# sanazkaviani/3d-latent-diffusion-model

Hardware: AMD Instinct MI355X
Metric: UNet denoising steps/sec (bf16, 1x4x24x24x24 latent; whole job = sum over GPUs) (higher is better)
Workload: dtype bf16

## Files before the change

### 3d-latent-diffusion-model_amd/_lib.py

```python
from __future__ import annotations

import ctypes as C
import os
import threading

LDM_MAX_LEVELS = 8
_HERE = os.path.dirname(os.path.abspath(__file__))
LIB_PATH = os.environ.get("LDM3D_LIB") or os.path.join(_HERE, "libldm3d.so")


class UNetCfg(C.Structure):
    _fields_ = [("spatial_dims", C.c_int), ("in_channels", C.c_int), ("out_channels", C.c_int),
                ("num_levels", C.c_int),
                ("channels", C.c_int * LDM_MAX_LEVELS), ("attention_levels", C.c_int * LDM_MAX_LEVELS),
                ("num_head_channels", C.c_int * LDM_MAX_LEVELS), ("num_res_blocks", C.c_int * LDM_MAX_LEVELS),
                ("norm_num_groups", C.c_int), ("norm_eps", C.c_float)]


class VaeCfg(C.Structure):
    _fields_ = [("spatial_dims", C.c_int), ("in_channels", C.c_int), ("out_channels", C.c_int),
                ("latent_channels", C.c_int), ("num_levels", C.c_int),
                ("channels", C.c_int * LDM_MAX_LEVELS), ("num_res_blocks", C.c_int * LDM_MAX_LEVELS),
                ("attention_levels", C.c_int * LDM_MAX_LEVELS),
                ("norm_num_groups", C.c_int), ("norm_eps", C.c_float),
# ... 139 lines not shown
    "ldm_op_conv3d_fin_gn": (C.c_int, [_P, C.c_int, _P, _P, _P, C.c_int, _P, _P, _P, C.c_int, C.c_float, C.c_int, _P, _P,
                                       C.c_int, C.c_int, C.c_int, C.c_int, C.c_int, C.c_int, C.c_int, C.c_int, _P, C.c_size_t, _P]),
    "ldm_op_group_norm_scratch_bytes": (C.c_size_t, [C.c_int, C.c_int, C.c_int]),
    "ldm_op_group_norm": (C.c_int, [_P, C.c_int, _P, C.c_int, _P, _P, C.c_int, C.c_float, C.c_int, _P, C.c_int, C.c_int,
                                    _P, C.c_size_t, _P]),
    "ldm_op_attention": (C.c_int, [_P, _P, C.c_int, C.c_int, C.c_int, _P]),
    "ldm_op_attention_hd": (C.c_int, [_P, _P, _P, C.c_int, C.c_int, C.c_int, C.c_int, _P]),
    "ldm_op_attention_bwd_hd": (C.c_int, [_P, _P, _P, _P, _P, _P, C.c_int, C.c_int, C.c_int, C.c_int, _P]),
    "ldm_op_attention_train": (C.c_int, [_P, _P, _P, C.c_int, C.c_int, C.c_int, _P]),
    "ldm_op_attention_bwd": (C.c_int, [_P, _P, _P, _P, _P, _P, C.c_int, C.c_int, C.c_int, _P]),
    "ldm_profile_start": (C.c_int, [C.c_int, C.c_int, C.c_int, C.c_int]),
    "ldm_profile_detail": (C.c_int, [C.POINTER(C.c_double), C.POINTER(C.c_double), C.c_int]),
    "ldm_profile_stop": (C.c_int, [C.POINTER(C.c_double)]),
    "ldm_set_plan_trace": (C.c_int, [C.c_char_p]),
    "ldm_op_pack_ncdhw_f32": (C.c_int, [_P, _P, C.c_int, C.c_int, C.c_int, C.c_int64, _P]),
    "ldm_op_unpack_ndhwc_f32": (C.c_int, [_P, _P, C.c_int, C.c_int, C.c_int, C.c_int64, _P]),
    "ldm_op_im2col_f32": (C.c_int, [_P, _P] + [C.c_int] * 10 + [_P]),
    "ldm_op_col2im_f32": (C.c_int, [_P, _P] + [C.c_int] * 10 + [_P]),
    "ldm_op_leaky_relu_f32": (C.c_int, [_P, _P, C.c_int64, C.c_float, _P]),
    "ldm_op_leaky_relu_bwd_f32": (C.c_int, [_P, _P, _P, C.c_int64, C.c_float, _P]),
    "ldm_op_gemm_f32": (C.c_int, [_P, C.c_int, _P, _P, _P, C.c_int64, C.c_int, C.c_int, C.c_int, _P]),
    "ldm_debug_conv_block_slots": (C.c_int, [C.c_int]),
    "ldm_op_conv3d_block_stats_rows": (C.c_int, [C.c_int, C.c_int, C.c_int, C.c_int]),
    "ldm_op_conv3d_block": (C.c_int, [_P, C.c_int, _P, _P, _P, C.c_int, _P, _P, _P, C.c_int, C.c_int, C.c_int, C.c_int, C.c_int, _P]),
    "ldm_op_conv3d_block128": (C.c_int, [_P, C.c_int, _P, _P, _P, C.c_int, _P, _P, _P, C.c_int, C.c_int, C.c_int, C.c_int, _P]),
    "ldm_op_linear_bf16": (C.c_int, [_P, C.c_int, _P, C.c_int, _P, _P, _P, _P, _P, C.c_int64, C.c_int, C.c_int, C.c_int, C.c_int,
                                     _P, C.c_int, C.c_int, _P, _P, C.c_int, C.c_float, C.c_int, _P, _P]),
    "ldm_op_linear_f32x3": (C.c_int, [_P, C.c_int, _P, C.c_int, _P, _P, _P, _P, _P, C.c_int64, C.c_int, C.c_int, C.c_int, _P]),
    "ldm_op_gemm_wgrad_f32": (C.c_int, [_P, C.c_int, _P, C.c_int, _P, C.c_int, C.c_int64, C.c_int, _P]),
    "ldm_op_group_norm_f32_scratch_bytes": (C.c_size_t, [C.c_int, C.c_int, C.c_int, C.c_int]),
    "ldm_op_group_norm_f32": (C.c_int, [_P, C.c_int, _P, _P, C.c_int, C.c_float, C.c_int, _P, C.c_int, C.c_int, _P, C.c_size_t, _P]),
    "ldm_op_group_norm_bwd_f32": (C.c_int, [_P, _P, C.c_int, _P, _P, C.c_int, C.c_float, C.c_int, _P, _P, _P, C.c_int, C.c_int, _P, C.c_size_t, _P]),
    "ldm_op_conv3d_f32_stats_blocks": (C.c_int, [C.c_int, C.c_int, C.c_int, C.POINTER(C.c_int)]),
    "ldm_op_conv3d_f32": (C.c_int, [_P, C.c_int, _P, C.c_int, _P, _P, _P, C.c_int, _P, _P, C.c_int, _P, _P] + [C.c_int] * 13
                          + [_P, C.c_size_t, _P]),
    "ldm_op_weight_flip_transpose_f32_ws_bytes": (C.c_size_t, [C.c_int, C.c_int, C.c_int]),
    "ldm_op_weight_flip_transpose_f32": (C.c_int, [_P, _P] + [C.c_int] * 6 + [_P, C.c_size_t, _P]),
    "ldm_op_conv3d_wgrad_f32": (C.c_int, [_P, C.c_int, _P, C.c_int, _P] + [C.c_int] * 13 + [_P]),
    "ldm_op_attention_f32": (C.c_int, [_P, _P, _P] + [C.c_int] * 5 + [_P]),
    "ldm_op_attention_bwd_f32": (C.c_int, [_P] * 6 + [C.c_int] * 4 + [_P]),
    "ldm_op_group_norm_bwd2_f32": (C.c_int, [_P, _P, C.c_int, _P, C.c_int, _P, _P, C.c_int, C.c_float, C.c_int, _P, _P, _P, _P, _P, _P,
                                             C.c_int, C.c_int, _P, C.c_size_t, _P]),
    "ldm_op_upsample_bwd_f32": (C.c_int, [_P, _P] + [C.c_int] * 5 + [_P]),
    "ldm_op_group_norm_bwd_saved_scratch_bytes": (C.c_size_t, [C.c_int] * 4),
    "ldm_op_group_norm_bwd_fold_chunks": (C.c_int, [C.c_int] * 4),
    "ldm_op_group_norm_bwd_saved": (C.c_int, [_P, _P, C.c_int, _P, C.c_int, _P, _P, _P, C.c_int, C.c_int] + [_P] * 7
                                    + [C.c_int] * 3 + [_P, C.c_size_t, _P]),
    "ldm_op_colsum_finalize_ws_bytes": (C.c_size_t, [_P, C.c_int]),
    "ldm_op_colsum_finalize": (C.c_int, [_P, _P, _P, C.c_int, C.c_int, _P, C.c_size_t, _P]),
    "ldm_op_grad_export_ws_bytes": (C.c_size_t, [_P, C.c_int]),
    "ldm_op_grad_export": (C.c_int, [_P, _P, _P, C.c_int, C.c_int, _P, C.c_size_t, _P]),
    "ldm_op_weight_flip_transpose_batched_ws_bytes": (C.c_size_t, [_P, C.c_int]),
    "ldm_op_weight_flip_transpose_batched": (C.c_int, [_P, _P, _P, C.c_int, _P, C.c_size_t, _P]),
    "ldm_op_linear_bwd_nz": (C.c_int, [C.c_int]),
    "ldm_op_linear_bwd": (C.c_int, [_P] * 6 + [C.c_int] * 6 + [_P, C.c_size_t, _P]),
    "ldm_op_upsample_bwd": (C.c_int, [_P, _P] + [C.c_int] * 5 + [_P]),
    "ldm_op_add_bf16": (C.c_int, [_P, _P, _P, C.c_int64, _P]),
    "ldm_op_vae_heads": (C.c_int, [_P] * 5 + [C.c_int] * 3 + [_P]),
    "ldm_op_vae_heads_bwd": (C.c_int, [_P, C.c_int] + [_P] * 5 + [C.c_int] * 5 + [_P]),
    "ldm_debug_kstamps": (C.c_int, [C.POINTER(C.c_uint64), C.c_int, C.c_int]),
    "ldm_model_plan_conv_cfgs": (C.c_int, [_P, C.c_char_p, C.c_int, C.c_int, C.c_int, C.c_int, C.POINTER(C.c_int), C.c_int]),
    "ldm_comm_unique_id": (C.c_int, [C.c_char_p]),
    "ldm_comm_init": (C.c_int, [C.c_int, C.c_int, C.c_char_p, C.POINTER(_P)]),
    "ldm_comm_init_custom": (C.c_int, [C.c_int, C.c_int, _P, _P, C.POINTER(_P)]),
    "ldm_comm_allreduce": (C.c_int, [_P, _P, C.c_int64, C.c_int, C.c_int, _P]),
    "ldm_comm_broadcast": (C.c_int, [_P, _P, C.c_int64, C.c_int, C.c_int, _P]),
    "ldm_comm_barrier": (C.c_int, [_P, _P]),
    "ldm_comm_destroy": (None, [_P]),
    "ldm_comm_rank": (C.c_int, [_P]),
    "ldm_comm_world": (C.c_int, [_P]),
    "ldm_model_set_grad_sync": (C.c_int, [_P, _P]),
    "ldm_model_set_grad_wire": (C.c_int, [_P, C.c_int]),
    "ldm_model_grad_sync_pending": (C.c_int, [_P]),
    "ldm_comm_stats": (C.c_int, [_P, C.POINTER(C.c_int64)]),
    "ldm_comm_is_rccl": (C.c_int, [_P]),
    "ldm_comm_rccl_version": (C.c_int, []),
    "ldm_model_plan_launches": (C.c_int, [_P, C.c_char_p, C.c_int, C.c_int, C.c_int, C.c_int]),
    "ldm_model_grad_sync_trace": (C.c_int, [_P, C.POINTER(C.c_double), C.POINTER(C.c_double), C.POINTER(C.c_int64), C.c_int]),
    "ldm_model_grad_schedule": (C.c_int, [_P, C.c_int, C.c_int, C.c_int, C.c_int, C.POINTER(C.c_int), C.POINTER(C.c_int64),
                                          C.POINTER(C.c_int64), C.POINTER(C.c_int), C.c_int]),
    "ldm_op_conv3d_thin": (C.c_int, [_P, C.c_int, _P, _P, _P] + [C.c_int] * 6 + [_P]),
    "ldm_op_conv3d_thin_f32_ws_bytes": (C.c_size_t, [C.c_int] * 6),
    "ldm_op_conv3d_thin_f32": (C.c_int, [_P, C.c_int, _P, _P, _P] + [C.c_int] * 6 + [_P, C.c_size_t, _P]),
    "ldm_op_timestep_embedding": (C.c_int, [_P, _P, C.c_int, C.c_int, _P]),
    "ldm_op_gemv": (C.c_int, [_P, C.c_int, _P, _P, _P] + [C.c_int] * 6 + [_P]),
    "ldm_op_pack2": (C.c_int, [_P, C.c_int, _P, C.c_int, _P, C.c_int, C.c_int, C.c_int64, C.c_int, C.c_int, C.c_float, _P]),
    "ldm_op_pack_im2col": (C.c_int, [_P, C.c_int, _P, C.c_int, _P] + [C.c_int] * 6 + [C.c_float, _P]),
    "ldm_op_phase_weights": (C.c_int, [_P, _P, C.c_int, C.c_int, _P]),
    "ldm_op_im2col_weights": (C.c_int, [_P, _P, C.c_int, C.c_int, C.c_int, C.c_int, _P]),
    "ldm_op_x3_weights": (C.c_int, [_P, _P, C.c_int64, C.c_int, _P]),
    "ldm_op_x3_phase_weights": (C.c_int, [_P, _P, C.c_int, C.c_int, _P]),
    "ldm_op_split_f32": (C.c_int, [_P, _P] + [C.c_int] * 6 + [_P]),
}
ALLREDUCE_FN = C.CFUNCTYPE(C.c_int, _P, _P, C.c_int64, C.c_int, C.c_int, _P)

_lib = None
_lock = threading.Lock()


class LdmError(RuntimeError):
    """Raised for every non-zero ldm_status (message from ldm_last_error)."""


def lib() -> C.CDLL:
    global _lib
    if _lib is None:
        with _lock:
            if _lib is None:
                if not os.path.exists(LIB_PATH):
                    raise LdmError(f"{LIB_PATH} not found: build it with `python -c 'import __graft_entry__ as g; "
                                   f"g.build()'` or `make -C {os.path.join(_HERE, 'csrc')}` (no CPU fallback exists)")
                h = C.CDLL(LIB_PATH)
                for name, (res, args) in SIGNATURES.items():
                    fn = getattr(h, name)
                    fn.restype = res
                    fn.argtypes = args
                _lib = h
    return _lib


def check(status: int) -> None:
    if status != 0:
        msg = lib().ldm_last_error()
        raise LdmError(f"libldm3d status {status}: {msg.decode() if msg else '?'}")


def ptr(t) -> int | None:
    return None if t is None else t.data_ptr()


def current_stream() -> int:
    import torch
    return torch.cuda.current_stream().cuda_stream
```

### 3d-latent-diffusion-model_amd/csrc/ldm3d.hip

```cpp
#include <hip/hip_runtime.h>
#include <dlfcn.h>
#include <math.h>
#include <stdarg.h>
#include <stdio.h>
#include <stdlib.h>
#include <string.h>

#include <algorithm>
#include <atomic>
#include <map>
#include <memory>
#include <string>
#include <type_traits>
#include <vector>

#include "../../include/ldm3d.h"
#include "attention.h"
#include "conv_igemm.h"
#include "conv_halo.h"
#include "conv_cube.h"
#include "conv_plane.h"
#ifdef LDM_EXPERIMENTS
#include "conv_halo_pp.h"
#include "conv_halo_rw.h"
// ... 51 lines not shown
        BLK_ATTR(8, 0, true)
#endif
#ifdef LDM_BLOCK_EXPERIMENTS
        BLK_ATTR(8, 1, false) BLK_ATTR(8, 2, false) BLK_ATTR(8, 4, false) BLK_ATTR(8, 3, false) BLK_ATTR(8, 7, false) BLK_ATTR(8, 8, false) BLK_ATTR(8, 15, false)
#endif
#undef BLK_ATTR
        attr_set = true;
    }
    const unsigned grid = (unsigned)tiles;
#ifdef LDM_BLOCK_EXPERIMENTS
#define BLK_DBG(D) if (TH == 8 && dbg == D) { hipLaunchKernelGGL((conv3_block_kernel<8, D, false>), dim3(grid), dim3(256), BlkGeom<8>::LDS_ALL, s, q); return hipGetLastError(); }
    BLK_DBG(1) BLK_DBG(2) BLK_DBG(4) BLK_DBG(3) BLK_DBG(7) BLK_DBG(8) BLK_DBG(15)
#undef BLK_DBG
#endif
    (void)dbg; (void)persist;
#ifdef LDM_EXPERIMENTS
    const long slots = g_block_slots > 0 ? g_block_slots : 2L * cus_tab[dev_];
    if (TH == 8 && persist && tiles > slots) { hipLaunchKernelGGL((conv3_block_kernel<8, 0, true>), dim3((unsigned)slots), dim3(256), BlkGeom<8>::LDS_ALL, s, q); return hipGetLastError(); }
#endif
    if (TH == 8) hipLaunchKernelGGL((conv3_block_kernel<8, 0, false>), dim3(grid), dim3(256), BlkGeom<8>::LDS_ALL, s, q);
    else hipLaunchKernelGGL((conv3_block_kernel<4, 0, false>), dim3(grid), dim3(256), BlkGeom<4>::LDS_ALL, s, q);
    return hipGetLastError();
}
static int device_cus() {
    static int tab[32] = {};
    int d = 0; if (hipGetDevice(&d) != hipSuccess || d < 0 || d >= 32) return 256;
    if (!tab[d]) { hipDeviceProp_t pr; tab[d] = (hipGetDeviceProperties(&pr, d) == hipSuccess && pr.multiProcessorCount >= 8) ? pr.multiProcessorCount : 256; }
    return tab[d];
}
static hipError_t launch_conv_block128(const BlockParams& q0, hipStream_t s) {
    BlockParams q = q0;
    q.td = (q.D + BLK_TD - 1) / BLK_TD; q.th = (q.H + 7) / 8; q.tw = (q.W + BLK_TW - 1) / BLK_TW;
    static bool attr_tab[32] = {}; bool& attr_set = attr_flag(attr_tab);
    if (!attr_set) {
        hipError_t e = hipFuncSetAttribute(reinterpret_cast<const void*>(&conv3_block128_kernel), hipFuncAttributeMaxDynamicSharedMemorySize, Blk128::LDS_ALL);
        if (e != hipSuccess) return e;
        attr_set = true;
    }
    hipLaunchKernelGGL(conv3_block128_kernel, dim3((unsigned)((long)q.N * q.td * q.th * q.tw)), dim3(512), Blk128::LDS_ALL, s, q);
    return hipGetLastError();
}
static inline int rup(int v, int m) { return (v + m - 1) / m * m; }
static inline size_t rup_sz(size_t v, size_t m) { return (v + m - 1) / m * m; }

static inline uint16_t host_f2bf(float f) {
    uint32_t u; memcpy(&u, &f, 4);
    if ((u & 0x7fffffffu) > 0x7f800000u) return (uint16_t)((u >> 16) | 0x40);
    u += 0x7fffu + ((u >> 16) & 1u);
    return (uint16_t)(u >> 16);
}

enum BaseId { BASE_NULL = 0, BASE_WS, BASE_W, BASE_IO0, BASE_IO1, BASE_IO2, BASE_IO3, BASE_IO4, BASE_IO5, BASE_W32, BASE_TAPO, BASE_TAPI, BASE_TTAB, BASE_SST, BASE_COUNT };
struct Ref { int base = BASE_NULL; size_t off = 0; };
static inline Ref ws_ref(size_t off) { Ref r; r.base = BASE_WS; r.off = off; return r; }
static inline Ref w_ref(size_t off) { Ref r; r.base = BASE_W; r.off = off; return r; }
static inline Ref io_ref(int i) { Ref r; r.base = BASE_IO0 + i; r.off = 0; return r; }
static inline Ref w32_ref(size_t off) { Ref r; r.base = BASE_W32; r.off = 2 * off; return r; }

struct Act {
    size_t off = 0; int C = 0; int N = 0, D = 0, H = 0, W = 0; bool valid = false;
    size_t stats_off = 0; bool has_stats = false;
    int stats_nrb = 0;
    int esz = 2;
    bool hl = false;
    size_t cs_off = 0; int cs_rows = 0;
    size_t bytes() const { return (size_t)N * D * H * W * C * esz; }
    long rows() const { return (long)N * D * H * W; }
};

enum OpKind { OP_PACK, OP_CONV, OP_FINALIZE, OP_GN_STATS, OP_GN_FINALIZE, OP_GN_PREP, OP_GN_APPLY, OP_ATTN, OP_SINUSOID,
              OP_GEMV, OP_VAE_HEADS, OP_GN_FUSED,
              OP_WT , OP_WT_BATCH, OP_WGRAD, OP_EXPORT , OP_EXPORT_BATCH, OP_COLSUM, OP_GNB, OP_ATTN_BWD, OP_ADD, OP_SUMPOOL, OP_LIN_DX, OP_LIN_DW, OP_VAE_HEADS_BWD,
              OP_GEMM_LIGHT,
              OP_COLSUM_BATCH,
              OP_IM2COL,
              OP_PACK32, OP_CONV32, OP_FIN32, OP_GN_STATS32, OP_GN_APPLY32, OP_ATTN32, OP_GEMV32,
              OP_TAP,
              OP_BUCKET, OP_BUCKET_JOIN,
              OP_UPS_SPLIT32,
              OP_CONV_THIN,
              OP_FIN_GN,
              OP_GEMM_LIGHT32,
              OP_CONV_BLOCK,
              OP_TEMB_ROW };

struct ConvCfg { int wgm, wgn, bk, splitk; int halo = 0, mtps = 0, qps = 0; int slab_lg = 0; int cube = 0; int th = 0, big = 0; int plane = 0; int wg = 0; };

struct ConvRec {
    Ref xa, xb, w; int ca, cb;
    Ref x1a, x1b, w1; int c1a, c1b;
    int N, Din, Hin, Win, Dout, Hout, Wout;
    int k, stride, pad, M;
    int couts, cout_pad, cout_real;
    int nchunk0, nchunk1, mtiles, ntiles;
    bool ups, exact;
    bool phase;
    bool x3;
    bool ep32_ndhwc, ep32_ncdhw;
    Ref bias, bias2, temb, residual; int temb_stride;
    Ref out; int f32_out;
    Ref partial, stats;
    int stats_nrb, stats_rows;
    Ref gamma, beta, gn_out; int gn_groups, gn_silu, gn_lg; float gn_eps;
    Ref gn_stats; int gn_nrb;
};

struct GnRec {
    Ref xa, xb; int ca, cb, N, DHW;
    Ref gamma, beta; int groups; float eps; bool silu;
    Ref stats_a, stats_b; int nrb_a, nrb_b;
    Ref partial; int nslab, rows_per_slab;
    Ref ab, mr;
    Ref out; bool out_hl;
    int rows_per_block, chunks;
    Ref dy, gsum, dgamma_n, dbeta_n;
    Ref cs; bool leaves_colsums;
    Ref acc_a, acc_b, dxa, dxb;
    int dgamma_flat, dbeta_flat;
    bool fp32;
    int count, out_stride; bool over_n;
};

struct WgradRec {
    Ref dy, x, dw; int cdy, cx;
    int Cout, Cin, dw_ld, dw_ci_off;
    int N, Din, Hin, Win, Dout, Hout, Wout;
    int ksize, stride, pad, ups, M;
    int ksplit, rows_total;
    bool fp32;
};

struct LayoutRec {
    Ref a, b, dst;
    int N, c_real, c_stored, D, H, W, DHW;
    bool internal;
    int esz, mode, ups;
    bool guided;
};

struct AttnRec {
    Ref qkv, out, lse;
    Ref d_o, delta, dqkv;
    int B, N, C, heads, d; float scale;
    bool x3, fp32;
};

struct LinRec {
    Ref w, bias, x, y;
    Ref dy, x_pre, dx, dW, db, part;
    int B, I, O, x_stride, y_stride, dy_stride;
    int silu, nz; bool fp32;
};

struct ElemRec {
    Ref a, b, out; int n;
    Ref ml, noise, mu, sigma, z;
    Ref dz, g_mu, g_sigma, dy; int c_dz;
    int N, D, H, W, C, L, DHW;
    bool fp32;
};

struct RangeRec { int first, end, count; bool fp32; };

struct Op {
    OpKind kind;
    ConvCfg cc;
    ConvRec cv;
    GnRec gn;
    WgradRec wg;
    LayoutRec lay;
    AttnRec at;
    LinRec lin;
    ElemRec el;
    RangeRec rg;
};

struct Pool {
    struct Blk { size_t off, size; };
    std::vector<Blk> free_list;
    std::map<size_t, size_t> live;
    size_t top = 0, high = 0;
    size_t alloc(size_t bytes) {
        bytes = rup_sz(bytes, 256);
// ... 191 lines not shown
        ConvW o = new_conv_slot(C, C, 1);
        reg_conv_into(p + ".attn.out_proj", o, C, C, 1, 0, true);
        convs[p + ".attn.out_proj"] = o;
    }
};

static int wgrad_ksplit(long M, int taps, int cout, int cin, bool hp = false, int stride = 1, int ups = 0);
static void conv32_cfg(long M, int cout_pad, int steps, bool x3, int* bn_out, int* sk_out);
static int fin32_stats_blocks(int N, int dhwo, int couts, int* rows);

static void gn_slabs(int N, int C, int DHW, int vec, int max_slabs, int* nslab, int* rps) {
    const int rows_par = std::max(1, 256 / std::max(1, C / vec));
    const int ns = std::min((DHW + rows_par - 1) / rows_par, std::max(1, max_slabs / N));
    *rps = (DHW + ns - 1) / ns;
    *nslab = (DHW + *rps - 1) / *rps;
}
static int gn_row_chunks(int N, int C, int DHW, int blocks, int row_multiple, int* rpb) {
    const int slices = (C + 63) / 64;
    const int chunks = std::max(1, std::min(blocks / (slices * N), (DHW + row_multiple - 1) / row_multiple));
    *rpb = rup((DHW + chunks - 1) / chunks, row_multiple);
    return (DHW + *rpb - 1) / *rpb;
}
static int gn_fused_blocks() { static const int v = ldm_xknob("LDM_GN_BLOCKS", 512); return v; }
static int gnb_fold_chunks(int N, int C, int groups, int DHW, int nslab, int* rpb) {
    if (C / groups > 64 || nslab > 512) return 0;
    return gn_row_chunks(N, C, DHW, 256, 32, rpb);
}
static int lin_dx_nz(int O) { return std::max(1, std::min(64, O / 64)); }
static int conv_out_size(int in, int k, int stride, int pad, int ups) {
    return ((in << ups) + ((stride == 2 && pad == 0 && k == 3) ? 1 : 2 * pad) - k) / stride + 1;
}
static int conv_mtiles(const ConvRec& c, const ConvCfg& cc) {
    const int bm = 64 * cc.wgm;
    if (cc.halo) return c.N * cc.mtps;
    if (c.phase) return c.N * 8 * (int)(((long)c.Din * c.Hin * c.Win + bm - 1) / bm);
    return (c.M + bm - 1) / bm;
}
static int splitk_stats_rows(int N, int dhw) { return N == 1 ? (dhw + 31) / 32 : dhw % 32 ? 0 : dhw / 32; }
static int conv_stats_rows(const ConvRec& c, const ConvCfg& cc) {
    const int dhwo = c.Dout * c.Hout * c.Wout, bm = 64 * cc.wgm;
    if (cc.splitk > 1) return splitk_stats_rows(c.N, dhwo);
    if (cc.plane) return c.Dout;
    if (cc.halo || c.phase) return conv_mtiles(c, cc) / c.N;
    return c.N == 1 ? (c.M + bm - 1) / bm : dhwo % bm ? 0 : dhwo / bm;
}

struct Builder {
    ldm_model* m; Plan* plan; Pool pool;
    size_t partial_off = 0, partial_bytes = 0;
    size_t gnpart_off = 0, gnpart_bytes = 0;
    size_t gnab_off = 0, gnab_bytes = 0;
    std::vector<size_t> partial_fixups, gnpart_fixups, gnab_fixups;
    std::string err;

    Act new_act(int N, int D, int H, int W, int C) {
        Act a; a.N = N; a.D = D; a.H = H; a.W = W; a.C = C; a.valid = true; a.esz = hp ? 4 : 2; a.off = pool.alloc(a.bytes()); return a;
    }
    bool hp = false;
    int tap_mode = 0;
    void tap(const std::string& name, Act& h, int c_real) {
        if (!tap_mode) return;
        TapInfo t; t.name = name; t.dims[0] = h.N; t.dims[1] = c_real; t.dims[2] = h.D; t.dims[3] = h.H; t.dims[4] = h.W; t.off = plan->tap_elems;
        plan->tap_elems += (size_t)h.N * c_real * h.D * h.H * h.W;
        Op o{}; o.kind = OP_TAP; LayoutRec& l = o.lay; l.a = ws_ref(h.off);
        l.dst.base = BASE_TAPO; l.dst.off = t.off * 4; l.b.base = BASE_TAPI; l.b.off = t.off * 4;
        l.N = h.N; l.c_real = c_real; l.c_stored = h.C; l.DHW = h.D * h.H * h.W; l.esz = h.esz; l.mode = tap_mode;
        plan->ops.push_back(o);
        plan->taps.push_back(t);
        if (tap_mode == 2 && h.has_stats) { pool.release(h.stats_off); h.has_stats = false; }
    }
    void pack(Ref src_a, Ref src_b, const Act& dst, int c_real, bool internal) {
        Op o{}; o.kind = hp ? OP_PACK32 : OP_PACK; LayoutRec& l = o.lay; l.a = src_a; l.b = src_b; l.dst = ws_ref(dst.off);
        l.N = dst.N; l.c_real = c_real; l.c_stored = dst.C; l.DHW = dst.D * dst.H * dst.W; l.internal = internal;
        l.guided = guided && !internal;
        plan->ops.push_back(o);
    }
    void free_act(Act& a) {
        if (train) return;
        if (a.valid) { pool.release(a.off); if (a.has_stats) pool.release(a.stats_off); }
        a.valid = false; a.has_stats = false;
    }
    bool train = false, recording = false;
    bool guided = false;

    struct ConvArgs {
        Act xa, xb;
        const ConvW* w = nullptr;
        int k = 3, stride = 1, pad = 1, ups = 0;
        int Do = 0, Ho = 0, Wo = 0;
        Act g1a, g1b; const ConvW* w1 = nullptr;
        Ref temb; int temb_stride = 0;
        Act residual;
        bool f32_out = false; Ref out_ref; int cout_real = 0;
        bool want_stats = true;
        Ref w_over; bool no_bias = false; int exact = 0;
        int temb_row = -1;
        int f32_tag = 0;
        const GnW* pre_gn = nullptr; int pre_groups = 0, pre_nrb = 0; float pre_eps = 0.f;
    };
    struct Tape {
        int kind = 0;
        ConvArgs c; Act out; bool leaf_input = false;
        const GnW* g = nullptr; Act xa, xb; size_t ab_off = 0, mr_off = 0; int groups = 0; bool silu = false;
        Act qkv, o; size_t lse_off = 0; int head_ch = 64;
    };
    std::vector<Tape> tape;

    static bool halo_enabled() { return ldm_knob("LDM_CONV_HALO", 1) != 0; }
    static int tall_mode() { return ldm_xknob("LDM_HALO_TALL", 2); }
    static bool light_enabled() { return ldm_knob("LDM_GEMM_LIGHT", 1) != 0; }
    static bool two_wg_enabled() { return ldm_knob("LDM_IGEMM_2WG", 1) != 0; }
    static bool phase_enabled() { return ldm_knob("LDM_CONV_PHASE", 1) != 0; }
    static bool halo_skip_enabled() { static const int v = ldm_knob("LDM_HALO_SKIP", 1); return v != 0; }
    static bool halo_skip_split_enabled() { static const int v = ldm_knob("LDM_HALO_SKIP_SPLIT", 1); return v != 0; }
    static bool cube_enabled() { return ldm_knob("LDM_CONV_CUBE", 1) != 0; }
    static bool cube_ok(int D, int H, int W, int cin0, int c1a, int c1b, int cout_pad) {
        return cube_enabled() && D >= 1 && H >= 1 && W >= 1 && D <= CUBE_EDGE && H <= CUBE_EDGE && W <= CUBE_EDGE && cin0 % 64 == 0 && cin0 >= 128 &&
               c1a % 64 == 0 && c1b % 64 == 0 && cout_pad % 16 == 0;
    }
    static ConvCfg cube_cfg(int cin0) { ConvCfg c{2, 2, 64, cin0 / 64}; c.cube = 1; return c; }
    static bool plane_enabled() { return ldm_knob("LDM_CONV_PLANE", 1) != 0; }
    static int plane_max_cin() { return (int)ldm_knob("LDM_CONV_PLANE_MAX_CIN", 256); }
    static bool plane_ok(int D, int H, int W, int cin0, int c1a, int c1b, int cout_pad) {
        return plane_enabled() && D >= 1 && H >= 1 && W >= 1 && D <= PLANE_EDGE && H <= PLANE_EDGE && W <= PLANE_EDGE &&
               (D > CUBE_EDGE || H > CUBE_EDGE || W > CUBE_EDGE) && cin0 % 64 == 0 && cin0 >= 128 && cin0 <= plane_max_cin() &&
               c1a % 64 == 0 && c1b % 64 == 0 && cout_pad % 16 == 0;
    }
    static ConvCfg plane_cfg() { ConvCfg c{2, 2, 64, 1}; c.plane = 1; return c; }
    static ConvCfg choose_cfg(long M, int cout_pad, int steps0, int bk, int halo_n = 0, long halo_dhw = 0, bool halo_only = false, int steps1 = 0) {
        ConvCfg best{2, 2, bk, 1}; double best_t = 1e30;
        const int steps = steps0 + steps1;
        const int rb = bk * 2;
        static const int splits[] = {1, 2, 3, 4, 6, 8, 9, 12, 16, 18, 24, 27, 32, 48, 64};
        for (int wgn = 1; wgn <= 4 && !halo_only; wgn *= 2) {
            const int bn = 64 * wgn, bm = 64 * (4 / wgn);
            if (cout_pad % bn) continue;
            const long tiles = ((M + bm - 1) / bm) * (cout_pad / bn);
            const double c_mfma = (double)bm * bn * bk * 2.0 / 4096.0;
            const double c_load = (double)(bm + bn) * rb / 28.0;
            const double c_step = std::max(c_mfma, c_load) + 60.0;
            for (int sk : splits) {
                if (sk > 1 && steps / sk < 6) break;
                const long nwg = tiles * sk;
                const int sps = (steps + sk - 1) / sk;
                const double rounds = ceil((double)nwg / 256.0);
                double t = rounds * (sps * c_step + 2500.0);
                if (sk > 1) t += 6000.0 + (double)M * cout_pad * 4.0 * sk * 2.0 / 2500.0;
                if (t < best_t) { best_t = t; best = ConvCfg{4 / wgn, wgn, bk, sk}; }
            }
        }
        if (halo_n > 0 && bk == 64 && cout_pad % 128 == 0 && halo_enabled()) {
            const int mtps = (int)((halo_dhw + 125) / 126), Q = steps0 / 3;
            const long tiles = (long)halo_n * mtps * (cout_pad / 128);
            const double c_mfma = 128.0 * 128.0 * 64.0 * 2.0 / 4096.0;
            const double c_load = (128.0 / 3.0 + 128.0) * 128.0 / 28.0;
            const double c_step = std::max(c_mfma, c_load) + 30.0;
            for (int sk : splits) {
                if (sk > 1 && Q / sk < 3) break;
                const int qps = (Q + sk - 1) / sk, skr = (Q + qps - 1) / qps;
                const long nwg = tiles * skr;
                const double rounds = ceil((double)nwg / 256.0);
                double t = rounds * (3.0 * qps * c_step + 2500.0 + ((steps1 + skr - 1) / skr) * 1.6 * c_step + (steps1 && skr > 1 ? 800.0 : 0.0));
                if (skr > 1) t += 6000.0 + (double)M * cout_pad * 4.0 * skr * 2.0 / 2500.0;
                if (steps1 && skr > 1 && !halo_skip_split_enabled()) continue;
                if (t < best_t) { best_t = t; best = ConvCfg{2, 2, 64, skr}; best.halo = 1; best.mtps = mtps; best.qps = qps; }
            }
        }
        if (halo_n > 0 && bk == 64 && cout_pad % 64 == 0 && halo_enabled() && tall_mode() != 0) {
            const int mtps = (int)((halo_dhw + 253) / 254), Q = steps0 / 3;
            const long tiles = (long)halo_n * mtps * (cout_pad / 64);
            const double c_mfma = 256.0 * 64.0 * 64.0 * 2.0 / 4096.0;
            const double c_load = (256.0 / 3.0 + 64.0) * 128.0 / 28.0;
            const double c_step = std::max(c_mfma, c_load) + 30.0;
            for (int sk : splits) {
                if (sk > 1 && Q / sk < 3) break;
                const int qps = (Q + sk - 1) / sk, skr = (Q + qps - 1) / qps;
                const long nwg = tiles * skr;
                const double rounds = ceil((double)nwg / 256.0);
                double t = rounds * (3.0 * qps * c_step + 2500.0 + ((steps1 + skr - 1) / skr) * 1.6 * c_step + (steps1 && skr > 1 ? 800.0 : 0.0));
                if (skr > 1) t += 6000.0 + (double)M * cout_pad * 4.0 * skr * 2.0 / 2500.0;
                if (steps1 && skr > 1 && !halo_skip_split_enabled()) continue;
                if (tall_mode() == 2 && cout_pad % 128 == 0) t = 1e31;
                if (tall_mode() == 3 && skr == 1 && best.halo == 1 && best.splitk == 1) t = 0.0;
                if (t < best_t) { best_t = t; best = ConvCfg{4, 1, 64, skr}; best.halo = 2; best.mtps = mtps; best.qps = qps; }
            }
        }
        return best;
    }
    static bool conv_halo_ok(const ConvRec& c, int bk, int forced_split) {
        return c.k == 3 && c.stride == 1 && c.pad == 1 && !c.ups && !c.exact && c.cb == 0 && bk == 64 &&
               c.Din == c.Dout && c.Hin == c.Hout && c.Win == c.Wout &&
               (c.c1a + c.c1b == 0 || (halo_skip_enabled() && (forced_split <= 1 || halo_skip_split_enabled())));
    }
    static void two_wg_steps(ConvCfg& cc, int steps, long mtiles, int cout_pad) {
        if (!cc.halo && !cc.plane && cc.bk == 64 && cc.wgm <= 2 && cc.splitk == 1 && two_wg_enabled() && steps <= 64 &&
            mtiles * (cout_pad / (64 * cc.wgn)) >= 512) cc.bk = 32;
    }
    static ConvCfg pick_cfg(const ConvRec& c, int bk, bool cube, bool plane, int wgn = 0, int splitk = 0) {
        const int cin0 = c.ca + c.cb, steps0 = c.k * c.k * c.k * (cin0 / bk), steps1 = (c.c1a + c.c1b) / bk;
        const long dhwo = (long)c.Dout * c.Hout * c.Wout;
        const bool halo_ok = conv_halo_ok(c, bk, splitk);
        ConvCfg cc = choose_cfg(c.M, c.cout_pad, steps0, bk, halo_ok ? c.N : 0, dhwo, false, steps1);
        if (cube && halo_ok && cube_ok(c.Dout, c.Hout, c.Wout, cin0, c.c1a, c.c1b, c.cout_pad)) cc = cube_cfg(cin0);
        else if (plane && halo_ok && plane_ok(c.Dout, c.Hout, c.Wout, cin0, c.c1a, c.c1b, c.cout_pad)) cc = plane_cfg();
        if (wgn) {
            const bool halo = halo_ok && halo_enabled();
            cc.wgn = wgn; cc.wgm = 4 / wgn; cc.halo = (wgn == 2 && halo && c.cout_pad % 128 == 0) ? 1 : (wgn == 1 && halo && tall_mode() != 0) ? 2 : 0;
        }
        if (splitk) cc.splitk = splitk;
        if (cc.halo) {
            const int Q = steps0 / 3;
            cc.qps = (Q + std::min(cc.splitk, Q) - 1) / std::min(cc.splitk, Q); cc.splitk = (Q + cc.qps - 1) / cc.qps;
            cc.mtps = (int)((dhwo + (cc.halo == 2 ? 253 : 125)) / (cc.halo == 2 ? 254 : 126));
        }
        if (!wgn && !splitk) two_wg_steps(cc, steps0 + steps1, conv_mtiles(c, cc), c.cout_pad);
        return cc;
    }

    static ConvRec conv_rec(const ConvArgs& a, int k, int stride, int pad, long M, int cout_real) {
        ConvRec c{}; c.N = a.xa.N; c.Din = a.xa.D; c.Hin = a.xa.H; c.Win = a.xa.W; c.Dout = a.Do; c.Hout = a.Ho; c.Wout = a.Wo;
        c.k = k; c.stride = stride; c.pad = pad; c.M = (int)M; c.couts = rup(a.w->cout, 32); c.cout_pad = a.w->cout_pad; c.cout_real = cout_real;
        return c;
    }
    static void conv_epilogue(ConvRec& c, const ConvArgs& a, const Act& out) {
        c.bias = a.no_bias ? Ref() : w_ref(a.w->b_off); c.temb = a.temb; c.temb_stride = a.temb_stride;
        c.residual = a.residual.valid ? ws_ref(a.residual.off) : Ref();
        c.out = a.f32_out ? a.out_ref : ws_ref(out.off); c.f32_out = a.f32_out ? 1 : 0;
    }
    static void conv_sources(ConvRec& c, const ConvArgs& a) {
        c.xa = ws_ref(a.xa.off); c.xb = a.xb.valid ? ws_ref(a.xb.off) : Ref(); c.ca = a.xa.C; c.cb = a.xb.valid ? a.xb.C : 0;
    }
    void record_conv(const ConvArgs& a, const Act& out) { if (recording) { Tape t; t.kind = 0; t.c = a; t.out = out; tape.push_back(t); } }
    static long thin_tiles(const ConvArgs& a) {
        return (long)a.xa.N * ((a.Do + THIN_TD - 1) / THIN_TD) * ((a.Ho + THIN_TH - 1) / THIN_TH) * ((a.Wo + THIN_TW - 1) / THIN_TW);
    }
    void emit_thin(const ConvArgs& a, long M, Ref w, int cout_real, bool x3) {
        Op op{}; op.kind = OP_CONV_THIN;
        ConvRec& c = op.cv; c = conv_rec(a, 3, 1, 1, M, cout_real); conv_epilogue(c, a, Act());
        c.xa = ws_ref(a.xa.off); c.ca = x3 ? 2 * a.xa.C : a.xa.C; c.x3 = x3; c.w = w;
        plan->ops.push_back(op);
    }
    Act emit_light(OpKind kind, const ConvArgs& a, long M, Ref w, int big, bool want_stats) {
        const int N = a.xa.N, rows = big ? 64 : 32;
        Op op{}; op.kind = kind; op.cc.big = big;
        ConvRec& c = op.cv; c = conv_rec(a, a.k, a.stride, a.pad, M, a.w->cout);
        op.cc.wg = kind == OP_GEMM_LIGHT && gemm_wg_ok(!a.xb.valid, a.xa.C + (a.xb.valid ? a.xb.C : 0), M);
        if (a.pre_gn) {
            op.cc.wg = 2; c.gamma = w_ref(a.pre_gn->g_off); c.beta = w_ref(a.pre_gn->b_off); c.gn_groups = a.pre_groups; c.gn_eps = a.pre_eps;
            c.gn_stats = ws_ref(a.xa.stats_off); c.gn_nrb = a.pre_nrb;
        }
        Act out = new_act(N, a.Do, a.Ho, a.Wo, c.couts);
        const long dhwo = (long)a.Do * a.Ho * a.Wo;
        if (want_stats && (N == 1 || dhwo % rows == 0)) {
            out.stats_off = pool.alloc((size_t)((M + rows - 1) / rows) * c.couts * 2 * 4); out.has_stats = true;
            out.stats_nrb = (int)(N == 1 ? (M + rows - 1) / rows : dhwo / rows);
        }
        conv_epilogue(c, a, out); conv_sources(c, a); c.w = w; c.stats = out.has_stats ? ws_ref(out.stats_off) : Ref();
        plan->ops.push_back(op);
        record_conv(a, out);
        return out;
    }
    Act emit_conv_block(const ConvArgs& a, long M, int th, int tiles) {
        const int N = a.xa.N;
        Op op{}; op.kind = OP_CONV_BLOCK; op.cc.th = th;
        ConvRec& c = op.cv; c = conv_rec(a, 3, 1, 1, M, a.w->cout);
        Act out = new_act(N, a.Do, a.Ho, a.Wo, c.couts);
        if (a.want_stats) { out.stats_off = pool.alloc((size_t)N * tiles * c.couts * 2 * 4); out.has_stats = true; out.stats_nrb = tiles; }
        conv_epilogue(c, a, out); conv_sources(c, a);
        c.w = a.w_over.base != BASE_NULL ? a.w_over : w_ref(a.w->w_off); c.stats = out.has_stats ? ws_ref(out.stats_off) : Ref();
        plan->ops.push_back(op);
        record_conv(a, out);
        return out;
    }
    void fin32_stats(Op& f, Act& out, const ConvArgs& a, int N, int dhwo, int couts) {
        static const int on = ldm_xknob("LDM_FIN32_STATS", 1);
        if (!on || train || !a.want_stats || a.f32_out || couts % 4 || couts > 1024) return;
        int rows = 0;
        const int nrb = fin32_stats_blocks(N, dhwo, couts, &rows);
        out.stats_off = pool.alloc((size_t)N * nrb * couts * 2 * 4); out.has_stats = true; out.stats_nrb = nrb;
        f.cv.stats = ws_ref(out.stats_off); f.cv.stats_nrb = nrb; f.cv.stats_rows = rows;
    }
    void fin32_x3(const ConvArgs& a, Act& out, int C, long M, int splitk, int ntiles) {
        Op f{}; f.kind = OP_FIN32; f.cc = ConvCfg{2, 2, 32, splitk};
        ConvRec& d = f.cv; d = conv_rec(a, 3, 1, 1, M, a.f32_out && a.cout_real ? a.cout_real : a.w->cout);
        conv_epilogue(d, a, out);
        d.w = w32_ref(a.w->w_off); d.ca = C; d.nchunk0 = C / 32; d.ntiles = ntiles; d.mtiles = (int)((M + 127) / 128);
        fin32_stats(f, out, a, a.xa.N, a.Do * a.Ho * a.Wo, d.couts);
        partial_fixups.push_back(plan->ops.size()); plan->ops.push_back(f);
    }
    Act conv32(const ConvArgs& a, const std::string& tag) {
        const ConvW& w = *a.w;
        if (a.w1) { err = "fp32 precision: unsupported conv form (" + tag + ")"; return Act(); }
        const int cin0 = a.xa.C + (a.xb.valid ? a.xb.C : 0);
        if (cin0 != w.cin_s || cin0 % 16 || a.xa.C % 16) { err = "conv " + tag + ": channel bookkeeping mismatch"; return Act(); }
        const int N = a.xa.N;
        const long M = (long)N * a.Do * a.Ho * a.Wo;
        if (M >= (1L << 31)) { err = "conv " + tag + ": M too large"; return Act(); }
        {
            static const int x3_phase = ldm_xknob("LDM_X3_PHASE", 1);
            const int C = a.xa.C;
            if (x3_phase && !train && a.ups == 1 && !a.exact && a.k == 3 && a.stride == 1 && a.pad == 1 && !a.xb.valid && !a.w1 && !a.f32_out &&
                a.w_over.base == BASE_NULL && !a.xa.hl && a.Do == 2 * a.xa.D && a.Ho == 2 * a.xa.H && a.Wo == 2 * a.xa.W && phase_enabled() &&
                w.x3p_off != (size_t)-1 && x3_halo_ok(w, M, C) && a.temb.base == BASE_NULL && !a.residual.valid) {
                Act sp = new_act(N, a.xa.D, a.xa.H, a.xa.W, C); sp.hl = true;
                Op u{}; u.kind = OP_UPS_SPLIT32; u.lay.a = ws_ref(a.xa.off); u.lay.dst = ws_ref(sp.off);
                u.lay.N = N; u.lay.c_stored = C; u.lay.D = a.xa.D; u.lay.H = a.xa.H; u.lay.W = a.xa.W; u.lay.ups = 0;
                plan->ops.push_back(u);
                Op op{}; op.kind = OP_CONV;
                ConvRec& c = op.cv; c = conv_rec(a, 2, 1, 1, M, w.cout);
                c.xa = ws_ref(sp.off); c.xb = ws_ref(sp.off); c.w = Ref{BASE_W32, 2 * m->arena_bytes + w.x3p_off};
                c.ca = 2 * C; c.cb = C; c.phase = c.x3 = true;
                const int steps0 = 8 * (3 * C / 64);
                ConvCfg cc = choose_cfg(M, w.cout_pad, steps0, 64);
                if (cc.wgm > 2 || cc.splitk != 1) cc = ConvCfg{2, 2, 64, 1};
                if (w.cout_pad % (64 * cc.wgn)) cc = ConvCfg{4, 1, 64, 1};
                two_wg_steps(cc, steps0, conv_mtiles(c, cc), w.cout_pad);
                op.cc = cc; c.nchunk0 = 3 * C / cc.bk;
                Act out = new_act(N, a.Do, a.Ho, a.Wo, rup(w.cout, 32));
                partial_bytes = std::max(partial_bytes, (size_t)M * w.cout_pad * 4);
                partial_fixups.push_back(plan->ops.size()); plan->ops.push_back(op);
                fin32_x3(a, out, C, M, 1, 1);
                free_act(sp);
// ... 43 lines not shown
                return out;
            }
            if (cc.splitk == 1 && x3_fused) {
                c.ep32_ndhwc = true; conv_epilogue(c, a, out);
                if (a.want_stats) {
                    out.stats_nrb = conv_stats_rows(c, cc);
                    out.stats_off = pool.alloc((size_t)N * out.stats_nrb * couts * 2 * 4); out.has_stats = true; c.stats = ws_ref(out.stats_off);
                }
                plan->ops.push_back(op);
                return out;
            }
            partial_bytes = std::max(partial_bytes, (size_t)cc.splitk * M * w.cout_pad * 4);
            partial_fixups.push_back(plan->ops.size()); plan->ops.push_back(op);
            fin32_x3(a, out, C, M, cc.splitk, w.cout_pad / 128 ? w.cout_pad / 128 : 1);
            return out;
        }
        static const int f32_x3 = ldm_knob("LDM_F32_X3", 1);
        const bool x3 = (f32_x3 == 2 || (f32_x3 == 1 && !train)) && cin0 % 32 == 0 && a.xa.C % 32 == 0;
        {
            static const int light_x3 = ldm_xknob("LDM_LIGHT_X3", 1);
            static const long light_x3_max_m = ldm_xknob("LDM_LIGHT_X3_MAX_M", 4096L);
            if (light_x3 && x3 && M <= light_x3_max_m && a.k == 1 && a.stride == 1 && a.pad == 0 && !a.ups && !a.exact && !a.f32_out && !a.xa.hl && a.temb.base == BASE_NULL &&
                (!a.xb.valid || a.xb.C % 32 == 0) && w.cout_pad % 32 == 0 && a.xa.D == a.Do && a.xa.H == a.Ho && a.xa.W == a.Wo &&
                M * (long)std::max(cin0, w.cout_pad) * 4 < (1L << 31)) {
                return emit_light(OP_GEMM_LIGHT32, a, M, a.w_over.base != BASE_NULL ? a.w_over : w32_ref(w.w_off), gemm_light_x3_big(M, w.cout_pad),
                                  a.want_stats && !train);
            }
        }
        const int kb = x3 ? 32 : 16;
        const int taps = a.k * a.k * a.k, nchunk = cin0 / kb, steps = taps * nchunk;
        const int mtiles = (int)((M + 127) / 128);
        int bn = 0, sk = 0;
        conv32_cfg(M, w.cout_pad, steps, x3, &bn, &sk);
        const int ntiles = (w.cout_pad + bn - 1) / bn;
        const int couts = a.f32_out ? 0 : rup(w.cout, 32);
        Act out;
        if (!a.f32_out) out = new_act(N, a.Do, a.Ho, a.Wo, couts);
        Op op{}; op.kind = OP_CONV32; op.cc = ConvCfg{2, bn / 64, kb, sk};
        ConvRec& c = op.cv; c = conv_rec(a, a.k, a.stride, a.pad, M, a.cout_real ? a.cout_real : w.cout);
        conv_epilogue(c, a, out); conv_sources(c, a);
        c.w = a.w_over.base != BASE_NULL ? a.w_over : w32_ref(w.w_off);
        c.ups = a.ups & 1; c.exact = a.exact & 1; c.nchunk0 = nchunk; c.mtiles = mtiles; c.ntiles = ntiles;
        if (sk > 1) { partial_bytes = std::max(partial_bytes, (size_t)sk * M * w.cout_pad * 4); partial_fixups.push_back(plan->ops.size()); }
        plan->ops.push_back(op);
        if (sk > 1) { Op f = op; f.kind = OP_FIN32; fin32_stats(f, out, a, N, a.Do * a.Ho * a.Wo, couts); partial_fixups.push_back(plan->ops.size()); plan->ops.push_back(f); }
        record_conv(a, out);
        return out;
    }

    Act conv(const ConvArgs& a, std::string tag = "") {
        if (hp) return conv32(a, tag);
        const ConvW& w = *a.w;
        const int cin0 = a.xa.C + (a.xb.valid ? a.xb.C : 0);
        int bk = 64;
        if (a.xa.C % 64 || (a.xb.valid && a.xb.C % 64)) bk = 32;
        int cin1 = 0;
        if (a.w1) {
            cin1 = a.g1a.C + (a.g1b.valid ? a.g1b.C : 0);
            if (a.g1a.C % 64 || (a.g1b.valid && a.g1b.C % 64)) bk = 32;
        }
        if (cin0 != w.cin_s || (a.w1 && cin1 != a.w1->cin_s) || cin0 % 32 || cin1 % 32) {
            err = "conv " + tag + ": channel bookkeeping mismatch"; return Act();
        }
        const int N = a.xa.N;
        const long M = (long)N * a.Do * a.Ho * a.Wo;
        {
            const long rows0 = (long)N * a.xa.D * a.xa.H * a.xa.W;
            const long big = std::max(std::max(rows0 * a.xa.C, a.xb.valid ? rows0 * a.xb.C : 0L),
                                      a.w1 ? std::max(M * a.g1a.C, a.g1b.valid ? M * a.g1b.C : 0L) : 0L) * 2;
            if (big >= (1L << 32)) { err = "conv " + tag + ": a source tensor exceeds 4 GiB (split the batch)"; return Act(); }
        }
        {
            static const int thin = ldm_knob("LDM_CONV_THIN", 1);
            static const long thin_min = ldm_knob("LDM_CONV_THIN_MIN", 512L);
            const int cr = a.cout_real ? a.cout_real : w.cout;
            if (thin && a.f32_out && a.k == 3 && a.stride == 1 && a.pad == 1 && !a.ups && !a.exact && !a.xb.valid && !a.w1 &&
                a.temb.base == BASE_NULL && !a.residual.valid && a.w_over.base == BASE_NULL && cr <= 4 && cin0 % 32 == 0 && cin0 <= 128 &&
                a.xa.D == a.Do && a.xa.H == a.Ho && a.xa.W == a.Wo &&
                thin_tiles(a) >= thin_min) {
                emit_thin(a, M, w_ref(w.w_off), cr, false);
                record_conv(a, Act());
                return Act();
            }
        }
        const bool phase = a.ups == 1 && !a.exact && a.k == 3 && a.stride == 1 && a.pad == 1 && !train && !a.xb.valid && !a.w1 &&
                           a.w_over.base == BASE_NULL && w.wp_off != 0 && phase_enabled() &&
                           a.Do == 2 * a.xa.D && a.Ho == 2 * a.xa.H && a.Wo == 2 * a.xa.W;
        if (gemm_light_ok(a.k, a.stride, a.ups, cin0, !a.w1, !a.f32_out && a.temb.base == BASE_NULL) && light_enabled() &&
            a.xa.D == a.Do && a.xa.H == a.Ho && a.xa.W == a.Wo && M * (long)cin0 * 2 < (1L << 31))
            return emit_light(OP_GEMM_LIGHT, a, M, a.w_over.base != BASE_NULL ? a.w_over : w_ref(w.w_off), gemm_light_big(M, w.cout_pad), a.want_stats);
        if (a.pre_gn) { err = "conv " + tag + ": a GroupNorm prologue needs the light GEMM"; return Act(); }
        if (conv_block_enabled() && a.k == 3 && a.stride == 1 && a.pad == 1 && a.ups == 0 && !a.exact && !a.xb.valid && !a.w1 && !a.f32_out &&
            w.cout_pad == 64 && rup(w.cout, 32) == 64 && cin0 <= conv_block_max_cin() &&
            a.xa.D == a.Do && a.xa.H == a.Ho && a.xa.W == a.Wo) {
            const int TH = conv_block_th();
            const int td = (a.Do + BLK_TD - 1) / BLK_TD, th = (a.Ho + TH - 1) / TH, tw = (a.Wo + BLK_TW - 1) / BLK_TW;
            static const long min_blocks = ldm_knob("LDM_CONV_BLOCK_MIN", 512L);
            if ((long)N * td * th * tw >= min_blocks) return emit_conv_block(a, M, TH, td * th * tw);
        }
        if (conv_block128_enabled() && a.k == 3 && a.stride == 1 && a.pad == 1 && a.ups == 0 && !a.exact && !a.xb.valid && !a.w1 && !a.f32_out &&
            w.cout_pad == 128 && rup(w.cout, 32) == 128 && cin0 <= conv_block128_max_cin() && a.xa.D == a.Do && a.xa.H == a.Ho && a.xa.W == a.Wo) {
            const int td = (a.Do + BLK_TD - 1) / BLK_TD, th = (a.Ho + 7) / 8, tw = (a.Wo + BLK_TW - 1) / BLK_TW;
            static const long min_blocks = ldm_knob("LDM_CONV_BLOCK128_MIN", 192L);
            static const long max_blocks = ldm_xknob("LDM_CONV_BLOCK128_MAX", 0L);
            const long tiles128 = (long)N * td * th * tw;
            if (tiles128 >= min_blocks && tiles128 <= (max_blocks > 0 ? max_blocks : (long)device_cus())) return emit_conv_block(a, M, 8, td * th * tw);
        }
        if (M >= (1L << 31)) { err = "conv " + tag + ": M too large"; return Act(); }
        Op op{}; op.kind = OP_CONV;
        ConvRec& c = op.cv; c = conv_rec(a, phase ? 2 : a.k, a.stride, a.pad, M, a.cout_real ? a.cout_real : w.cout);
        conv_sources(c, a);
        c.w = a.w_over.base != BASE_NULL ? a.w_over : w_ref(phase ? w.wp_off : w.w_off);
        if (a.w1) {
            c.x1a = ws_ref(a.g1a.off); c.c1a = a.g1a.C; c.w1 = w_ref(a.w1->w_off); c.bias2 = w_ref(a.w1->b_off);
            if (a.g1b.valid) { c.x1b = ws_ref(a.g1b.off); c.c1b = a.g1b.C; }
        }
        c.phase = phase; c.ups = !phase && (a.ups & 1); c.exact = !phase && (a.exact & 1);
        const ConvCfg cc = op.cc = pick_cfg(c, bk, !train && !phase, !train && !phase && !a.f32_out);
        c.nchunk0 = cin0 / cc.bk; c.nchunk1 = cin1 / cc.bk;
        Act out;
        if (!a.f32_out) {
            out = new_act(N, a.Do, a.Ho, a.Wo, c.couts);
            const int nrb = a.want_stats ? conv_stats_rows(c, cc) : 0;
            if (a.want_stats && cc.splitk > 1) { out.stats_off = pool.alloc((size_t)((M + 31) / 32) * c.couts * 2 * 4); out.has_stats = true; }
            else if (nrb > 0) { out.stats_off = pool.alloc((size_t)N * nrb * c.couts * 2 * 4); out.has_stats = true; out.stats_nrb = nrb; }
        }
        conv_epilogue(c, a, out);
        c.stats = out.has_stats ? ws_ref(out.stats_off) : Ref();
        if (cc.splitk > 1) { partial_bytes = std::max(partial_bytes, (size_t)cc.splitk * M * w.cout_pad * 4); partial_fixups.push_back(plan->ops.size()); }
        plan->ops.push_back(op);
        if (cc.splitk > 1) { Op f = op; f.kind = OP_FINALIZE; partial_fixups.push_back(plan->ops.size()); plan->ops.push_back(f); }
        record_conv(a, out);
        return out;
    }

    static bool fin_gn_enabled() { static const int v = ldm_knob("LDM_FIN_GN", 1); return v != 0; }
    std::map<size_t, Act> prenorm;
    bool fuse_fin_gn(Act& raw, bool keep_raw, const GnW& g, int groups, float eps, bool silu, Act* y) {
        if (hp || train || !fin_gn_enabled() || plan->ops.size() < 2 || !raw.valid) return false;
        Op& f = plan->ops.back();
        Op& cv = plan->ops[plan->ops.size() - 2];
        if (f.kind != OP_FINALIZE || cv.kind != OP_CONV || f.cv.f32_out || f.cv.out.base != BASE_WS || f.cv.out.off != raw.off) return false;
        const int C = raw.C, N = raw.N, DHW = raw.D * raw.H * raw.W;
        if (C != g.C || !fin_gn_ok(C, groups, DHW) || f.cv.phase) return false;
        const int lg = fin_gn_lg(C, groups);
        static const long max_kb = ldm_knob("LDM_FIN_GN_MAX_KB", 400);
        if ((long)cv.cc.splitk * DHW * (C / groups) * 4 > max_kb * 1024) return false;
        if (f.cv.cout_pad % (1 << lg)) return false;
        Act out = new_act(N, raw.D, raw.H, raw.W, C);
        f.kind = OP_FIN_GN;
        f.cv.gamma = w_ref(g.g_off); f.cv.beta = w_ref(g.b_off); f.cv.gn_out = ws_ref(out.off);
        f.cv.stats = Ref();
        f.cv.gn_groups = groups; f.cv.gn_silu = silu ? 1 : 0; f.cv.gn_lg = lg; f.cv.gn_eps = eps;
        f.cc.slab_lg = lg; cv.cc.slab_lg = lg; cv.cv.stats = Ref();
        if (raw.has_stats) { pool.release(raw.stats_off); raw.has_stats = false; }
        if (!keep_raw) { f.cv.out = Ref(); pool.release(raw.off); raw.valid = false; }
        *y = out;
        return true;
    }

    static bool x3_halo_ok(const ConvW& w, long rows, int C) {
        static const int on = ldm_xknob("LDM_X3_HALO", 1);
        static const long min_rows = ldm_xknob("LDM_X3_HALO_ROWS", 1L);
        static const int f32_x3 = ldm_knob("LDM_F32_X3", 1);
        return on && f32_x3 != 0 && halo_enabled() && w.k == 3 && w.x3_off != (size_t)-1 && C == w.cin_s && C % 64 == 0 && rows >= min_rows &&
               rows * C * 4 < (1L << 32);
// ... 447 lines not shown

    size_t temb_all_off = 0; int tproj_stride = 0;

    void finish() {
        size_t top = rup_sz(pool.high, 256);
        partial_off = top; top += rup_sz(partial_bytes, 256);
        gnpart_off = top; top += rup_sz(gnpart_bytes, 256);
        gnab_off = top; top += rup_sz(gnab_bytes, 256);
        pool.high = top;
        for (size_t k : partial_fixups) plan->ops[k].cv.partial = ws_ref(partial_off);
        for (size_t k : gnpart_fixups) plan->ops[k].gn.partial = ws_ref(gnpart_off);
        for (size_t k : gnab_fixups) plan->ops[k].gn.ab = ws_ref(gnab_off);
        plan->ws_bytes = pool.high + 256;
    }
};

static int unet_register(ldm_model* m) {
    const ldm_unet_cfg& c = m->ucfg;
    const int L = c.num_levels; const int* ch = c.channels;
    const int temb = ch[0] * 4;
    for (int i = 0; i < L; ++i) if (ch[i] % 32 || ch[i] % c.norm_num_groups)
        return fail(LDM_ERR_UNSUPPORTED, "UNet channels must be multiples of 32 and of norm_num_groups (level %d: %d)", i, ch[i]);
    std::vector<std::pair<std::string, int>> tprojs;
    bool collect = true;
    auto reg_res = [&](const std::string& p, int cin, int cout) {
        if (collect) { tprojs.push_back({p, cout}); return; }
        m->reg_gn(p + ".norm1", cin);
        m->reg_conv(p + ".conv1", cin, cin, cout, 3);
        m->reg_gn(p + ".norm2", cout);
        m->reg_conv(p + ".conv2", cout, cout, cout, 3);
        if (cin != cout) m->reg_conv(p + ".skip_connection", cin, cin, cout, 1);
    };
    auto walk = [&]() {
    if (!collect) { m->reg_conv("conv_in", c.in_channels, rup(c.in_channels, 32), ch[0], 3); m->reg_im2col("conv_in", c.in_channels); }
    int oc = ch[0];
    for (int i = 0; i < L; ++i) {
        int ic = oc; oc = ch[i];
        for (int j = 0; j < c.num_res_blocks[i]; ++j) {
            char p[96]; snprintf(p, sizeof p, "down_blocks.%d.resnets.%d", i, j);
            reg_res(p, j == 0 ? ic : oc, oc);
            if (c.attention_levels[i] && !collect) { snprintf(p, sizeof p, "down_blocks.%d.attentions.%d", i, j); m->reg_attn(p, oc); }
        }
        if (i != L - 1 && !collect) { char p[96]; snprintf(p, sizeof p, "down_blocks.%d.downsampler.op", i); m->reg_conv(p, oc, oc, oc, 3); }
    }
    reg_res("middle_block.resnet_1", ch[L - 1], ch[L - 1]);
    if (!collect) m->reg_attn("middle_block.attention", ch[L - 1]);
    reg_res("middle_block.resnet_2", ch[L - 1], ch[L - 1]);
    oc = ch[L - 1];
    for (int i = 0; i < L; ++i) {
        const int lvl = L - 1 - i;
        int prev = oc; oc = ch[lvl];
        const int ic = ch[std::max(lvl - 1, 0)];
        const int nres = c.num_res_blocks[lvl] + 1;
        for (int j = 0; j < nres; ++j) {
            const int skip_c = (j == nres - 1) ? ic : oc;
            const int rin = (j == 0) ? prev : oc;
            char p[96]; snprintf(p, sizeof p, "up_blocks.%d.resnets.%d", i, j);
            reg_res(p, rin + skip_c, oc);
            if (c.attention_levels[lvl] && !collect) { snprintf(p, sizeof p, "up_blocks.%d.attentions.%d", i, j); m->reg_attn(p, oc); }
        }
        if (i != L - 1 && !collect) { char p[96]; snprintf(p, sizeof p, "up_blocks.%d.upsampler.postconv", i); m->reg_conv(p, oc, oc, oc, 3, true); }
    }
    if (!collect) { m->reg_gn("out.0", ch[0]); m->reg_conv("out.2", ch[0], ch[0], c.out_channels, 3); }
    };
    walk();
    m->reg_linear("time_embed.0", ch[0], temb);
    m->reg_linear("time_embed.2", temb, temb);
    int rows = 0; for (auto& t : tprojs) rows += t.second;
    m->tproj_rows = rows;
    m->tproj_w_off = m->arena_alloc((size_t)rows * temb * 2);
    m->tproj_b_off = m->arena_alloc((size_t)rows * 4);
    int r = 0;
    for (auto& t : tprojs) {
        m->tproj_row[t.first] = r;
        m->reg_linear_at(t.first + ".time_emb_proj", temb, t.second, m->tproj_w_off + (size_t)r * temb * 2, m->tproj_b_off + (size_t)r * 4);
        r += t.second;
    }
    collect = false;
    walk();
    return 0;
}

static int unet_build(ldm_model* m, int B, int D, int H, int W, Plan* plan, bool train, bool hp = false, int tap_mode = 0, bool temb_table = false,
                      bool guided = false) {
    const ldm_unet_cfg& c = m->ucfg;
    const int L = c.num_levels; const int* ch = c.channels;
    const int temb = ch[0] * 4, G = c.norm_num_groups; const float eps = c.norm_eps;
    if (train && tap_mode) return fail(LDM_ERR_UNSUPPORTED, "debug taps are inference-only");
    Builder b; b.m = m; b.plan = plan; b.train = train; b.recording = train; b.hp = hp; b.tap_mode = tap_mode; b.guided = guided;
    const size_t sin_off = b.pool.alloc((size_t)B * ch[0] * 4);
    const size_t e1_off = b.pool.alloc((size_t)B * temb * 4);
    const size_t e2_off = b.pool.alloc((size_t)B * temb * 4);
    b.tproj_stride = m->tproj_rows;
    b.temb_all_off = b.pool.alloc(((size_t)B * m->tproj_rows + 256) * 4);
    const LinW& l0 = m->lins.at("time_embed.0"); const LinW& l2 = m->lins.at("time_embed.2");
    if (temb_table && !train) {
        Op o{}; o.kind = OP_TEMB_ROW; o.lin.y = ws_ref(b.temb_all_off); o.lin.O = m->tproj_rows; o.lin.B = B; plan->ops.push_back(o);
    } else {
    { Op o{}; o.kind = OP_SINUSOID; o.lin.x = io_ref(2); o.lin.y = ws_ref(sin_off); o.lin.B = B; o.lin.O = ch[0];
      plan->ops.push_back(o); }
    auto gemv = [&](size_t w_off, size_t b_off, size_t x_off, size_t y_off, int I, int O, int xs, int ys, int silu) {
        Op o{}; o.kind = hp ? OP_GEMV32 : OP_GEMV; LinRec& l = o.lin;
        l.w = hp ? w32_ref(w_off) : w_ref(w_off); l.bias = w_ref(b_off); l.x = ws_ref(x_off); l.y = ws_ref(y_off);
        l.I = I; l.O = O; l.x_stride = xs; l.y_stride = ys; l.silu = silu; l.B = B; plan->ops.push_back(o);
    };
    gemv(l0.w_off, l0.b_off, sin_off, e1_off, ch[0], temb, ch[0], temb, 0);
    gemv(l2.w_off, l2.b_off, e1_off, e2_off, temb, temb, temb, temb, 1);
    gemv(m->tproj_w_off, m->tproj_b_off, e2_off, b.temb_all_off, temb, m->tproj_rows, temb, m->tproj_rows, 1);
    }

    const int cin_s = rup(c.in_channels, 32);
    Act h = b.conv_in_im2col("conv_in", io_ref(0), io_ref(1), B, D, H, W, c.in_channels, false);
    if (!h.valid) {
        if (!b.err.empty()) return fail(LDM_ERR_UNSUPPORTED, "%s", b.err.c_str());
        Act xin = b.new_act(B, D, H, W, cin_s);
        b.pack(io_ref(0), io_ref(1), xin, c.in_channels, false);
        h = b.conv3("conv_in", xin);
        if (train && !b.tape.empty()) b.tape.back().leaf_input = true;
        b.free_act(xin);
    }
    if (!h.valid) return fail(LDM_ERR_UNSUPPORTED, "%s", b.err.c_str());
    b.tap("conv_in", h, ch[0]);
    std::vector<Act> skips; skips.push_back(h);
    char p[96];
    for (int i = 0; i < L; ++i) {
        for (int j = 0; j < c.num_res_blocks[i]; ++j) {
            snprintf(p, sizeof p, "down_blocks.%d.resnets.%d", i, j);
            char pa[96]; snprintf(pa, sizeof pa, "down_blocks.%d.attentions.%d.norm", i, j);
            Act hn = b.resblock(p, h, Act(), ch[i], G, eps, ".skip_connection", true, c.attention_levels[i] ? &m->gns.at(pa) : nullptr);
            if (!hn.valid) return fail(LDM_ERR_UNSUPPORTED, "%s", b.err.c_str());
            b.tap(p, hn, ch[i]);
            if (c.attention_levels[i]) {
                snprintf(p, sizeof p, "down_blocks.%d.attentions.%d", i, j);
                Act ha = b.attention(p, hn, c.num_head_channels[i], G, eps);
                b.free_act(hn);
                if (!ha.valid) return fail(LDM_ERR_UNSUPPORTED, "%s", b.err.c_str());
                hn = ha;
                b.tap(p, hn, ch[i]);
            }
            skips.push_back(hn); h = hn;
        }
        if (i != L - 1) {
            if ((h.D | h.H | h.W) & 1) return fail(LDM_ERR_UNSUPPORTED, "odd spatial size %dx%dx%d at a UNet downsample", h.D, h.H, h.W);
            snprintf(p, sizeof p, "down_blocks.%d.downsampler.op", i);
            Act hd = b.conv3(p, h, 2, 1);
            if (!hd.valid) return fail(LDM_ERR_UNSUPPORTED, "%s", b.err.c_str());
            b.tap(p, hd, ch[i]);
            skips.push_back(hd); h = hd;
        }
    }
    {
        Act h1 = b.resblock("middle_block.resnet_1", h, Act(), ch[L - 1], G, eps, ".skip_connection", true, &m->gns.at("middle_block.attention.norm"));
        if (!h1.valid) return fail(LDM_ERR_UNSUPPORTED, "%s", b.err.c_str());
        b.tap("middle_block.resnet_1", h1, ch[L - 1]);
        Act h2 = b.attention("middle_block.attention", h1, c.num_head_channels[L - 1], G, eps);
        b.free_act(h1);
        if (!h2.valid) return fail(LDM_ERR_UNSUPPORTED, "%s", b.err.c_str());
        b.tap("middle_block.attention", h2, ch[L - 1]);
        Act h3 = b.resblock("middle_block.resnet_2", h2, Act(), ch[L - 1], G, eps, ".skip_connection", true);
        b.free_act(h2);
        if (!h3.valid) return fail(LDM_ERR_UNSUPPORTED, "%s", b.err.c_str());
        b.tap("middle_block.resnet_2", h3, ch[L - 1]);
        h = h3;
    }
    for (int i = 0; i < L; ++i) {
        const int lvl = L - 1 - i;
        for (int j = 0; j < c.num_res_blocks[lvl] + 1; ++j) {
            Act s = skips.back(); skips.pop_back();
            snprintf(p, sizeof p, "up_blocks.%d.resnets.%d", i, j);
            char pa[96]; snprintf(pa, sizeof pa, "up_blocks.%d.attentions.%d.norm", i, j);
            Act hn = b.resblock(p, h, s, ch[lvl], G, eps, ".skip_connection", true, c.attention_levels[lvl] ? &m->gns.at(pa) : nullptr);
            b.free_act(h); b.free_act(s);
// ... 189 lines not shown
    Act first = b.conv_in_im2col("encoder.blocks.0", io_ref(0), Ref(), B, D, H, W, c.in_channels, true);
    if (first.valid) {
        b.tap("encoder.blocks.0", first, c.channels[0]);
        LDM_TRY(vae_run_layout(b, "encoder", ae_encoder_layout(c), first, c.norm_num_groups, c.norm_eps, false, 0, &h, 1));
    } else {
        if (!b.err.empty()) return fail(LDM_ERR_UNSUPPORTED, "%s", b.err.c_str());
        Act xin = b.new_act(B, D, H, W, cs);
        b.pack(io_ref(0), Ref(), xin, c.in_channels, false);
        LDM_TRY(vae_run_layout(b, "encoder", ae_encoder_layout(c), xin, c.norm_num_groups, c.norm_eps, false, 0, &h));
    }
    const int dhw = h.D * h.H * h.W;
    const size_t ml_off = b.pool.alloc((size_t)B * 2 * c.latent_channels * dhw * 4);
    Builder::ConvArgs a; a.xa = h; a.w = &m->convs.at("quant_heads"); a.k = 1; a.pad = 0; a.Do = h.D; a.Ho = h.H; a.Wo = h.W;
    a.f32_out = true; a.out_ref = ws_ref(ml_off); a.cout_real = 2 * c.latent_channels;
    b.conv(a, "quant_heads");
    if (!b.err.empty()) return fail(LDM_ERR_UNSUPPORTED, "%s", b.err.c_str());
    b.free_act(h);
    { Op o{}; o.kind = OP_VAE_HEADS; ElemRec& e = o.el; e.ml = ws_ref(ml_off); e.noise = io_ref(1); e.mu = io_ref(2); e.sigma = io_ref(3); e.z = io_ref(4);
      e.N = B; e.L = c.latent_channels; e.DHW = dhw; plan->ops.push_back(o); }
    b.finish();
    return 0;
}

static int vae_build_decode(ldm_model* m, int B, int d, int h_, int w, Plan* plan, bool hp = false, int tap_mode = 0) {
    const ldm_vae_cfg& c = m->vcfg;
    Builder b; b.m = m; b.plan = plan; b.hp = hp; b.tap_mode = tap_mode;
    const int ls = rup(c.latent_channels, 32);
    Act zin = b.new_act(B, d, h_, w, ls);
    b.pack(io_ref(0), Ref(), zin, c.latent_channels, false);
    Builder::ConvArgs a; a.xa = zin; a.w = &m->convs.at("post_quant_conv"); a.k = 1; a.pad = 0; a.Do = d; a.Ho = h_; a.Wo = w;
    Act z2 = b.conv(a, "post_quant_conv");
    b.free_act(zin);
    if (!z2.valid) return fail(LDM_ERR_UNSUPPORTED, "%s", b.err.c_str());
    b.tap("post_quant_conv", z2, c.latent_channels);
    Act out;
    LDM_TRY(vae_run_layout(b, "decoder", ae_decoder_layout(c), z2, c.norm_num_groups, c.norm_eps, true, 1, &out));
    b.finish();
    return 0;
}

static int vae_build_train(ldm_model* m, int B, int D, int H, int W, Plan* plan, bool hp = false) {
    const ldm_vae_cfg& c = m->vcfg;
    Builder b; b.m = m; b.plan = plan; b.train = true; b.recording = true; b.hp = hp;
    const int cs = rup(c.in_channels, 32), L = c.latent_channels, ls = rup(L, 32);
    Act xin = b.new_act(B, D, H, W, cs);
    b.pack(io_ref(0), Ref(), xin, c.in_channels, true);
    const size_t t0 = b.tape.size();
    Act h;
    LDM_TRY(vae_run_layout(b, "encoder", ae_encoder_layout(c), xin, c.norm_num_groups, c.norm_eps, false, 0, &h));
    if (b.tape.size() > t0) b.tape[t0].leaf_input = true;
    const int dhw = h.D * h.H * h.W;
    const size_t ml_off = b.pool.alloc((size_t)B * 2 * L * dhw * 4), z_off = b.pool.alloc((size_t)B * L * dhw * 4);
    { Builder::ConvArgs a; a.xa = h; a.w = &m->convs.at("quant_heads"); a.k = 1; a.pad = 0; a.Do = h.D; a.Ho = h.H; a.Wo = h.W;
      a.f32_out = true; a.out_ref = ws_ref(ml_off); a.cout_real = 2 * L; a.f32_tag = 1;
      b.conv(a, "quant_heads"); }
    if (!b.err.empty()) return fail(LDM_ERR_UNSUPPORTED, "%s", b.err.c_str());
    { Op o{}; o.kind = OP_VAE_HEADS; ElemRec& e = o.el; e.ml = ws_ref(ml_off); e.noise = io_ref(1); e.mu = io_ref(2); e.sigma = io_ref(3); e.z = ws_ref(z_off);
      e.N = B; e.L = L; e.DHW = dhw; plan->ops.push_back(o); }
    Act zin = b.new_act(B, h.D, h.H, h.W, ls);
    b.pack(ws_ref(z_off), Ref(), zin, L, true);
    Builder::ConvArgs pq; pq.xa = zin; pq.w = &m->convs.at("post_quant_conv"); pq.k = 1; pq.pad = 0; pq.Do = h.D; pq.Ho = h.H; pq.Wo = h.W;
    Act z2 = b.conv(pq, "post_quant_conv");
    if (!z2.valid) return fail(LDM_ERR_UNSUPPORTED, "%s", b.err.c_str());
    Act out;
    LDM_TRY(vae_run_layout(b, "decoder", ae_decoder_layout(c), z2, c.norm_num_groups, c.norm_eps, true, 5, &out));
    plan->train = true; plan->bwd_begin = plan->ops.size();
    b.recording = false;
    b.vae_zin = zin; b.vae_ml_off = ml_off; b.vae_z_off = z_off; b.vae_L = L;
    { Op o{}; o.kind = OP_WT_BATCH; o.rg.fp32 = hp; plan->ops.push_back(o); }
    const int cos_ = rup(c.out_channels, 32);
    Act dout = b.new_act(B, D, H, W, cos_);
    b.pack(io_ref(0), Ref(), dout, c.out_channels, true);
    b.bucket_hi = b.done_from = m->flat_total;
    if (!b.backward_all(dout)) return fail(LDM_ERR_UNSUPPORTED, "%s", b.err.c_str());
    b.done_from = 0; b.close_bucket(true);
    { Op o{}; o.kind = OP_BUCKET_JOIN; plan->ops.push_back(o); }
    if (plan->wt_tab.upload(b.wt_descs, b.wt_map) || plan->exp_tab.upload(b.exp_descs, b.exp_map) ||
        (!b.cs_descs.empty() && plan->cs_tab.upload(b.cs_descs, b.cs_map)))
        return fail(LDM_ERR_HIP, "descriptor table upload failed");
    b.finish();
    return 0;
}

struct Bases { char* p[BASE_COUNT]; int sampler_steps; float guide_fill; };
static inline char* rp(const Bases& b, const Ref& r) { return r.base == BASE_NULL ? nullptr : (b.p[r.base] ? b.p[r.base] + r.off : nullptr); }

static int xcd_rows_mode() { static const int v = ldm_xknob("LDM_XCD_ROWS", 0); return v; }
static inline int conv_tile_order(const ConvParams& p) { return (xcd_rows_mode() && p.splitk == 1 && !p.phase_mode) ? 1 : 0; }

template <int WGM, int WGN, int BK>
static int launch_conv_t(const ConvParams& p_in, hipStream_t s) {
    ConvParams p = p_in; p.tile_order = conv_tile_order(p);
    constexpr int STAGE = (64 * WGM + 64 * WGN) * BK * 2;
    constexpr int NG = (BK == 64) ? 2 : 1;
    constexpr int NS = (STAGE * 4 <= 131072) ? 4 : 3;
    constexpr int LDS = NS * STAGE + 28 * 64 * WGM * 4;
    static bool attr_tab[32] = {}; bool& attr_set = attr_flag(attr_tab);
    if (!attr_set) {
        HIP_TRY(hipFuncSetAttribute(reinterpret_cast<const void*>(&conv_igemm_kernel<WGM, WGN, BK, NS, NG>),
                                    hipFuncAttributeMaxDynamicSharedMemorySize, LDS));
        attr_set = true;
    }
    const int grid = p.mtiles * p.ntiles * p.splitk;
    hipLaunchKernelGGL((conv_igemm_kernel<WGM, WGN, BK, NS, NG>), dim3(grid), dim3(256 * NG), LDS, s, p);
    return 0;
}

struct ProfState {
    bool on = false; int wgm = 0, wgn = 0, bk = 0, halo = 0;
    std::vector<hipEvent_t> ev; size_t used = 0;
    std::vector<double> flops;
    double flops_all = 0.0; long launches_all = 0;
};
static ProfState g_prof;

static double conv_algorithmic_flops(const ConvParams& p) {
    const double taps = (double)p.ksize * p.ksize * p.ksize;
    return 2.0 * (double)p.M * (double)p.CoutReal * (taps * (double)(p.c0a + p.c0b) + (double)(p.c1a + p.c1b));
}

static void launch_finalize(const FinalizeParams& f, bool wt, hipStream_t s) {
    const dim3 grid((f.M + 31) / 32, (f.CoutS + 63) / 64);
    if (wt) hipLaunchKernelGGL(splitk_finalize_kernel<true>, grid, dim3(256), 0, s, f);
    else hipLaunchKernelGGL(splitk_finalize_kernel<false>, grid, dim3(256), 0, s, f);
}
static int launch_conv_impl(const ConvParams& p, const ConvCfg& cc, hipStream_t s);
static int launch_conv(const ConvParams& p, const ConvCfg& cc, hipStream_t s) {
    if (!g_prof.on) return launch_conv_impl(p, cc, s);
    g_prof.flops_all += conv_algorithmic_flops(p); g_prof.launches_all++;
    const bool hit = cc.wgm == g_prof.wgm && cc.wgn == g_prof.wgn && cc.bk == g_prof.bk && cc.halo == g_prof.halo &&
                     g_prof.used + 2 <= g_prof.ev.size();
    if (hit) HIP_TRY(hipEventRecord(g_prof.ev[g_prof.used], s));
    LDM_TRY(launch_conv_impl(p, cc, s));
    if (hit) { HIP_TRY(hipEventRecord(g_prof.ev[g_prof.used + 1], s)); g_prof.used += 2; g_prof.flops.push_back(conv_algorithmic_flops(p)); }
    return 0;
}

static int launch_conv_halo(const ConvParams& p_in, hipStream_t s, bool tall = false) {
    ConvParams p = p_in; p.tile_order = conv_tile_order(p);
    fastdiv_make((unsigned)(p.Hout * p.Wout), &p.fd_hw_m, &p.fd_hw_s); fastdiv_make((unsigned)p.Wout, &p.fd_w_m, &p.fd_w_s);
    constexpr int LDS = 6 * 16384 + 3 * 16384 + 9 * 128 * 4;
    constexpr int LDS_TALL = 6 * 8192 + 3 * 32768 + 9 * 256 * 4;
    static bool attr_tab[32] = {}; bool& attr_set = attr_flag(attr_tab);
    if (!attr_set) {
        HIP_TRY(hipFuncSetAttribute(reinterpret_cast<const void*>(&conv3_halo_kernel<6>), hipFuncAttributeMaxDynamicSharedMemorySize, LDS));
        HIP_TRY(hipFuncSetAttribute(reinterpret_cast<const void*>(&conv3_halo_kernel<6, 0, true>), hipFuncAttributeMaxDynamicSharedMemorySize, LDS_TALL));
        HIP_TRY(hipFuncSetAttribute(reinterpret_cast<const void*>(&conv3_halo_kernel<6, 0, false, true>), hipFuncAttributeMaxDynamicSharedMemorySize, LDS));
        HIP_TRY(hipFuncSetAttribute(reinterpret_cast<const void*>(&conv3_halo_kernel<6, 0, true, true>), hipFuncAttributeMaxDynamicSharedMemorySize, LDS_TALL));
        attr_set = true;
    }
    static const int persist = ldm_xknob("LDM_HALO_PERSIST", 1);
    static int cus_tab[32] = {};
    int dev_ = 0; if (hipGetDevice(&dev_) != hipSuccess || dev_ < 0 || dev_ >= 32) dev_ = 0;
    int& cus = cus_tab[dev_];
    if (!cus) { hipDeviceProp_t pr; if (hipGetDeviceProperties(&pr, dev_) == hipSuccess) cus = pr.multiProcessorCount; if (cus < 8) cus = 256; cus -= cus % 8; }
    const int tiles = p.mtiles * p.ntiles * p.splitk;
    const int grid = (persist && tiles > cus) ? cus : tiles;
    const bool loop = grid < tiles;
    static const int mi = ldm_knob("LDM_HALO_MASK_INLINE", 1);
    if (mi) {
        static bool mi_attr_tab[32] = {}; bool& mi_attr = attr_flag(mi_attr_tab);
        if (!mi_attr) {
            HIP_TRY(hipFuncSetAttribute(reinterpret_cast<const void*>(&conv3_halo_kernel<6, 0, false, false, true>), hipFuncAttributeMaxDynamicSharedMemorySize, LDS));
            HIP_TRY(hipFuncSetAttribute(reinterpret_cast<const void*>(&conv3_halo_kernel<6, 0, true, false, true>), hipFuncAttributeMaxDynamicSharedMemorySize, LDS_TALL));
            mi_attr = true;
        }
    }
// ... 325 lines not shown
}

static bool wt_stores() { static const int v = ldm_xknob("LDM_WT_STORES", 1); return v != 0; }
template <class P> static void launch_gn_fused(P p, int chunks, hipStream_t s) {
    p.xcd_rows = xcd_rows_mode();
    const dim3 grid(chunks, (p.ca + p.cb + 63) / 64, p.N);
    if (wt_stores()) hipLaunchKernelGGL(gn_fused_apply_kernel<true>, grid, dim3(256), 0, s, p);
    else hipLaunchKernelGGL(gn_fused_apply_kernel<false>, grid, dim3(256), 0, s, p);
}

static ConvParams conv_params_geom(const ConvRec& c, const ConvCfg& cc) {
    ConvParams p{};
    p.c0a = c.ca; p.c0b = c.cb; p.c1a = c.c1a; p.c1b = c.c1b;
    p.N = c.N; p.Din = c.Din; p.Hin = c.Hin; p.Win = c.Win; p.Dout = c.Dout; p.Hout = c.Hout; p.Wout = c.Wout;
    p.ksize = c.k; p.stride = c.stride; p.pad = c.pad; p.ups = c.ups; p.exact = c.exact; p.M = c.M;
    p.mtiles = conv_mtiles(c, cc); p.ntiles = c.cout_pad / (64 * cc.wgn); p.halo_mtps = cc.mtps; p.q_per_split = cc.qps;
    p.phase_mode = c.phase; p.mtiles_pp = c.phase ? p.mtiles / (8 * c.N) : 0;
    if (c.x3) { p.x3_n = (c.ca / 2) / 64; p.raw_partial = (c.ep32_ndhwc || c.ep32_ncdhw) ? 0 : 1; }
    p.CoutS = c.couts; p.CoutPad = c.cout_pad; p.CoutReal = c.cout_real; p.nchunk0 = c.nchunk0; p.nchunk1 = c.nchunk1;
    p.steps0 = c.k * c.k * c.k * c.nchunk0; p.steps1 = c.nchunk1;
    p.splitk = cc.splitk; p.steps_per_split = cc.halo ? 3 * cc.qps : (p.steps0 + p.steps1 + p.splitk - 1) / p.splitk;
    p.temb_stride = c.temb_stride; p.slab_lg = cc.slab_lg;
    return p;
}
static ConvParams conv_params(const Op& o, const Bases& bs) {
    const ConvRec& c = o.cv; ConvParams p = conv_params_geom(c, o.cc);
    p.x0a = (const bf16_t*)rp(bs, c.xa); p.x0b = (const bf16_t*)rp(bs, c.xb); p.w0 = (const bf16_t*)rp(bs, c.w);
    p.x1a = (const bf16_t*)rp(bs, c.x1a); p.x1b = (const bf16_t*)rp(bs, c.x1b); p.w1 = (const bf16_t*)rp(bs, c.w1);
    p.zero_page = (const bf16_t*)bs.p[BASE_W];
    p.bias = (const float*)rp(bs, c.bias); p.bias2 = (const float*)rp(bs, c.bias2); p.temb = (const float*)rp(bs, c.temb);
    if (c.ep32_ndhwc) { p.out32 = (float*)rp(bs, c.out); p.residual32 = (const float*)rp(bs, c.residual); }
    else {
        p.residual = (const bf16_t*)rp(bs, c.residual);
        if (c.f32_out) p.out_f32 = (float*)rp(bs, c.out); else p.out = (bf16_t*)rp(bs, c.out);
    }
    p.partial = (float*)rp(bs, c.partial); p.stats = (float*)rp(bs, c.stats);
    return p;
}
static Conv32Params conv32_params(const Op& o, const Bases& bs) {
    const ConvRec& c = o.cv; Conv32Params p{};
    p.xa = (const float*)rp(bs, c.xa); p.xb = (const float*)rp(bs, c.xb); p.ca = c.ca; p.cb = c.cb; p.w = (const float*)rp(bs, c.w);
    p.N = c.N; p.Din = c.Din; p.Hin = c.Hin; p.Win = c.Win; p.Dout = c.Dout; p.Hout = c.Hout; p.Wout = c.Wout;
    p.ksize = c.k; p.stride = c.stride; p.pad = c.pad; p.ups = c.ups; p.exact = c.exact; p.M = c.M;
    p.CoutS = c.couts; p.CoutPad = c.cout_pad; p.CoutReal = c.cout_real; p.nchunk = c.nchunk0; p.steps = c.k * c.k * c.k * c.nchunk0;
    p.splitk = o.cc.splitk; p.steps_per_split = (p.steps + p.splitk - 1) / p.splitk; p.mtiles = c.mtiles; p.ntiles = c.ntiles;
    p.bias = (const float*)rp(bs, c.bias); p.temb = (const float*)rp(bs, c.temb); p.temb_stride = c.temb_stride; p.residual = (const float*)rp(bs, c.residual);
    if (c.f32_out) p.out_ncdhw = (float*)rp(bs, c.out); else p.out = (float*)rp(bs, c.out);
    p.partial = (float*)rp(bs, c.partial);
    if (c.stats_nrb > 0) { p.stats = (float*)rp(bs, c.stats); p.stats_nrb = c.stats_nrb; p.stats_rows = c.stats_rows; }
    return p;
}
static FinalizeParams finalize_params(const ConvParams& p) {
    FinalizeParams f{}; f.partial = p.partial; f.splitk = p.splitk; f.M = p.M; f.CoutPad = p.CoutPad; f.CoutS = p.CoutS; f.CoutReal = p.CoutReal;
    f.DHWo = p.Dout * p.Hout * p.Wout; f.bias = p.bias; f.bias2 = p.bias2; f.temb = p.temb; f.temb_stride = p.temb_stride; f.residual = p.residual;
    f.out = p.out; f.out_f32 = p.out_f32; f.stats = p.stats;
    return f;
}
template <class P> static P wgrad_params(const WgradRec& w, const Bases& bs) {
    P p{}; p.dy = (decltype(p.dy))rp(bs, w.dy); p.cdy = w.cdy; p.x = (decltype(p.x))rp(bs, w.x); p.cx = w.cx;
    p.dw = (float*)rp(bs, w.dw); p.Cout = w.Cout; p.Cin = w.Cin; p.dw_ld = w.dw_ld; p.dw_ci_off = w.dw_ci_off;
    p.N = w.N; p.Din = w.Din; p.Hin = w.Hin; p.Win = w.Win; p.Dout = w.Dout; p.Hout = w.Hout; p.Wout = w.Wout;
    p.ksize = w.ksize; p.stride = w.stride; p.pad = w.pad; p.ups = w.ups; p.M = w.M;
    p.co_tiles = (p.Cout + 127) / 128; p.ci_tiles = (p.Cin + 127) / 128; p.ksplit = w.ksplit;
    p.slab_stride = (long)w.ksize * w.ksize * w.ksize * w.rows_total * w.dw_ld;
    return p;
}
template <class P> static P attn_params(const AttnRec& a, const Bases& bs) {
    P p{}; p.qkv = (decltype(p.qkv))rp(bs, a.qkv); p.out = (decltype(p.out))rp(bs, a.out); p.lse = (float*)rp(bs, a.lse);
    p.B = a.B; p.N = a.N; p.C = a.C; p.heads = a.heads; p.d = a.d; p.scale = a.scale;
    return p;
}
template <class P> static P attn_bwd_params(const AttnRec& a, const Bases& bs) {
    P p{}; p.qkv = (decltype(p.qkv))rp(bs, a.qkv); p.o = (decltype(p.o))rp(bs, a.out); p.d_o = (decltype(p.d_o))rp(bs, a.d_o);
    p.lse = (const float*)rp(bs, a.lse); p.delta = (float*)rp(bs, a.delta); p.dqkv = (decltype(p.dqkv))rp(bs, a.dqkv);
    p.B = a.B; p.N = a.N; p.C = a.C; p.d = a.d; p.heads = a.heads; p.scale = a.scale;
    return p;
}

struct PlanTrace { bool on = false; std::string path; PlanTrace() { const char* e = getenv("LDM_PLAN_TRACE"); if (e && *e) { on = true; path = e; } } };
static PlanTrace g_plan_trace;
struct LaneCtx { GradSyncState* sync = nullptr; };
static void guided_layout_launch(OpKind kind, const LayoutRec& l, const float* x, int cx, const float* cond, int cc, float fill, void* dst, hipStream_t s);
static void guided_combine_launch(const float* u, const float* c, float w, float* out, int64_t n, hipStream_t s);

static int run_plan(const Plan& plan, const Bases& bs, const int* rt, hipStream_t s, size_t begin = 0, size_t end = (size_t)-1,
                    LaneCtx lanes = LaneCtx()) {
    if (end > plan.ops.size()) end = plan.ops.size();
    const char* trace_path = g_plan_trace.on ? g_plan_trace.path.c_str() : nullptr;
    std::vector<hipEvent_t> tev;
    if (trace_path) { tev.resize(end - begin + 1); for (auto& e : tev) HIP_TRY(hipEventCreate(&e)); }
    struct TraceDone {
        const Plan& plan; size_t begin, end; std::vector<hipEvent_t>& ev; hipStream_t s; const char* path;
        ~TraceDone() {
            if (ev.empty()) return;
            (void)hipEventRecord(ev.back(), s); (void)hipEventSynchronize(ev.back());
            FILE* f = fopen(path, "a");
            for (size_t oi = begin; oi < end && f; ++oi) {
                const Op& o = plan.ops[oi]; float ms = 0.f; (void)hipEventElapsedTime(&ms, ev[oi - begin], ev[oi - begin + 1]);
                fprintf(f, "%zu,%zu,%d,%.3f", plan.ops.size(), oi, (int)o.kind, ms * 1e3f);
                const ConvRec& c = o.cv;
                if (o.kind == OP_CONV || o.kind == OP_FINALIZE)
                    fprintf(f, ",M=%d k=%d s=%d ups=%d cin=%d+%d(x%d) cin1=%d couts=%d cfg=%dx%dx%d splitk=%d halo=%d mtps=%d qps=%d cube=%d", c.M, c.k, c.stride,
                            c.ups | c.exact << 1 | c.phase << 2 | c.x3 << 3 | c.ep32_ndhwc << 4 | c.ep32_ncdhw << 5, c.ca, c.cb, c.nchunk0, c.c1a + c.c1b, c.couts,
                            o.cc.wgm, o.cc.wgn, o.cc.bk, o.cc.splitk, o.cc.plane ? 6 : o.cc.halo, o.cc.mtps, o.cc.qps, o.cc.cube);
                else {
                    const GnRec& g = o.gn; const WgradRec& w = o.wg; const LayoutRec& l = o.lay; const AttnRec& at = o.at;
                    const LinRec& li = o.lin; const ElemRec& el = o.el; const RangeRec& r = o.rg;
                    int v[6] = {};
                    auto six = [&](int a, int b, int c2, int d, int e, int h) { v[0] = a; v[1] = b; v[2] = c2; v[3] = d; v[4] = e; v[5] = h; };
                    switch (o.kind) {
                        case OP_FIN_GN: six(c.gn_groups, c.gn_silu, c.gn_lg, c.c1b, c.N, c.Din); break;
                        case OP_CONV32: case OP_FIN32: six(c.ca, c.cb, c.stats_nrb, c.stats_rows, c.N, c.Din); break;
                        case OP_CONV_THIN: six(c.N, c.Din, c.Hin, c.Win, c.x3 ? c.ca / 2 * 3 : c.ca, c.cout_pad); break;
                        case OP_CONV_BLOCK: six(c.N, c.Dout, c.Hout, c.Wout, c.ca, o.cc.th); break;
                        case OP_GEMM_LIGHT: case OP_GEMM_LIGHT32: six(c.M, c.ca + c.cb, c.couts, c.cout_pad, o.cc.big, c.ca); break;
                        case OP_GN_STATS: case OP_GN_STATS32: six(g.ca, g.cb, g.DHW, g.nslab, g.rows_per_slab, g.N); break;
                        case OP_GN_FINALIZE: six(g.nslab, g.ca + g.cb, g.groups, g.DHW, g.N, 0); break;
                        case OP_GN_PREP: six(g.ca, g.cb, g.nrb_a, g.groups, g.DHW, g.N); break;
                        case OP_GN_FUSED: six(g.ca, g.cb, g.nrb_a, g.nrb_b, g.groups, g.DHW); break;
                        case OP_GN_APPLY: six(g.ca, g.cb, g.DHW, g.N, g.silu, 0); break;
                        case OP_GN_APPLY32: six(g.ca, g.cb, g.DHW, g.N, g.silu, g.nrb_a ? 1 : g.nslab); break;
                        case OP_COLSUM: six(g.N, g.nslab, g.ca, g.over_n, g.count, g.out_stride); break;
                        case OP_GNB: six(g.ca, g.cb, g.groups, g.DHW, g.N, g.silu); break;
                        case OP_WGRAD: six(w.cdy, w.cx, w.Cout, w.Cin, w.dw_ld, w.dw_ci_off); break;
                        case OP_PACK: case OP_PACK32: six(l.N, l.c_real, l.c_stored, l.DHW, l.internal, 0); break;
                        case OP_IM2COL: six(l.N, l.c_real, l.c_stored, l.D, l.H, l.W); break;
                        case OP_UPS_SPLIT32: six(l.N, l.c_stored, l.D, l.H, l.W, l.ups); break;
                        case OP_TAP: six(l.N, l.c_real, l.c_stored, l.DHW, l.esz, l.mode); break;
                        case OP_ATTN: case OP_ATTN32: six(at.B, at.N, at.C, at.heads, at.d, at.x3); break;
                        case OP_ATTN_BWD: six(at.B, at.N, at.C, at.d, at.fp32, 0); break;
                        case OP_SINUSOID: six(li.B, li.O, 0, 0, 0, 0); break;
                        case OP_TEMB_ROW: six(li.O, li.B, 0, 0, 0, 0); break;
                        case OP_GEMV: case OP_GEMV32: six(li.I, li.O, li.x_stride, li.y_stride, li.silu, li.B); break;
                        case OP_LIN_DX: case OP_LIN_DW: six(li.B, li.I, li.O, li.dy_stride, li.x_stride, li.silu); break;
                        case OP_VAE_HEADS: six(el.N, el.L, el.DHW, 0, 0, 0); break;
                        case OP_VAE_HEADS_BWD: six(el.N, el.L, el.C, el.DHW, el.c_dz, el.fp32); break;
                        case OP_ADD: six(el.n, el.fp32, 0, 0, 0, 0); break;
                        case OP_SUMPOOL: six(el.N, el.D, el.H, el.W, el.C, el.fp32); break;
                        case OP_WT_BATCH: six(r.fp32, 0, 0, 0, 0, 0); break;
                        case OP_COLSUM_BATCH: case OP_EXPORT_BATCH: six(r.first, r.end, 0, 0, 0, 0); break;
                        case OP_BUCKET: six(r.first, r.count, 0, 0, 0, 0); break;
                        case OP_BUCKET_JOIN: case OP_WT: case OP_EXPORT: case OP_CONV: case OP_FINALIZE: break;
                    }
                    fprintf(f, ",i=%d %d %d %d %d %d", v[0], v[1], v[2], v[3], v[4], v[5]);
                }
                fprintf(f, "\n");
            }
            if (f) fclose(f);
            for (auto e : ev) (void)hipEventDestroy(e);
        }
    } trace_done{plan, begin, end, tev, s, trace_path};
    for (size_t oi = begin; oi < end; ++oi) {
        const Op& o = plan.ops[oi];
        if (trace_path) HIP_TRY(hipEventRecord(tev[oi - begin], s));
        switch (o.kind) {
            case OP_PACK: case OP_PACK32: case OP_IM2COL: {
                const LayoutRec& l = o.lay;
                int cx = rt[0], cc = rt[1];
                if (l.internal) { cx = l.c_real; cc = 0; }
                if (cx + cc != l.c_real) return fail(LDM_ERR_BAD_ARG, "x_channels + cond_channels = %d, model expects %d", cx + cc, l.c_real);
                const float* xa = (const float*)rp(bs, l.a); const float* xb = (const float*)rp(bs, l.b);
                if (l.guided) {
                    if (cc < 1 || !xb || (l.N & 1)) return fail(LDM_ERR_BAD_ARG, "a guided plan needs a condition tensor");
                    guided_layout_launch(o.kind, l, xa, cx, xb, cc, bs.guide_fill, rp(bs, l.dst), s);
                } else
                if (o.kind == OP_IM2COL) launch_pack_im2col(xa, cx, xb, cc, (bf16_t*)rp(bs, l.dst), l.N, l.D, l.H, l.W, l.c_stored, s);
                else launch_pack2(xa, cx, xb, cc, rp(bs, l.dst), l.N, l.c_stored, l.DHW, o.kind == OP_PACK32, s);
                break; }
            case OP_CONV_THIN: {
                const ConvRec& c = o.cv;
                ThinParams q{}; q.x = (const bf16_t*)rp(bs, c.xa); q.w = (const bf16_t*)rp(bs, c.w); q.bias = (const float*)rp(bs, c.bias);
                q.out = (float*)rp(bs, c.out); q.N = c.N; q.D = c.Din; q.H = c.Hin; q.W = c.Win; q.CoutPad = c.cout_pad; q.CoutReal = c.cout_real;
                if (c.x3) { q.x3_c = c.ca / 2; q.Cin = 3 * q.x3_c; } else q.Cin = c.ca;
                if (!q.w) return fail(LDM_ERR_NOT_LOADED, "the weight arena is empty");
                HIP_TRY(launch_conv_thin(q, s));
                break; }
            case OP_CONV_BLOCK: {
                const ConvRec& c = o.cv;
                BlockParams q{}; q.x = (const bf16_t*)rp(bs, c.xa); q.w = (const bf16_t*)rp(bs, c.w); q.bias = (const float*)rp(bs, c.bias);
                q.temb = (const float*)rp(bs, c.temb); q.temb_stride = c.temb_stride; q.residual = (const bf16_t*)rp(bs, c.residual); q.out = (bf16_t*)rp(bs, c.out);
                q.stats = (float*)rp(bs, c.stats); q.N = c.N; q.D = c.Dout; q.H = c.Hout; q.W = c.Wout; q.Cin = c.ca;
                if (!q.w) return fail(LDM_ERR_NOT_LOADED, "the weight arena is empty");
                if (c.couts == 128) HIP_TRY(launch_conv_block128(q, s)); else HIP_TRY(launch_conv_block(q, o.cc.th, s));
                break; }
            case OP_UPS_SPLIT32: {
                const LayoutRec& l = o.lay;
                launch_split_f32((const float*)rp(bs, l.a), (bf16_t*)rp(bs, l.dst), l.N, l.c_stored, l.D, l.H, l.W, l.ups, s);
                break; }
            case OP_CONV32: case OP_FIN32: {
                const Conv32Params p = conv32_params(o, bs);
                if (!p.w) return fail(LDM_ERR_NOT_LOADED, "fp32 precision: the fp32 weight arena is empty (re-upload the parameters after ldm_model_set_precision)");
                if (o.kind == OP_CONV32) launch_conv32(p, o.cc.bk == 32, o.cc.wgn * 64, s);
                else launch_fin32(p, s);
                break; }
            case OP_GEMM_LIGHT32: {
                const ConvRec& c = o.cv;
                LightX3Params p{};
                p.x = (const float*)rp(bs, c.xa); p.xb = (const float*)rp(bs, c.xb); p.ca = c.ca;
                p.w = (const float*)rp(bs, c.w);
                if (!p.w) return fail(LDM_ERR_NOT_LOADED, "fp32 precision: the fp32 weight arena is empty (re-upload the parameters after ldm_model_set_precision)");
                p.bias = (const float*)rp(bs, c.bias); p.residual = (const float*)rp(bs, c.residual);
                p.out = (float*)rp(bs, c.out); p.stats = (float*)rp(bs, c.stats);
                p.M = c.M; p.K = c.ca + c.cb; p.CoutS = c.couts;
                HIP_TRY(launch_gemm_light_x3(p, c.cout_pad, o.cc.big, s));
                break; }
            case OP_GN_STATS32: {
                const GnRec& g = o.gn;
                Gn32Params p{}; p.xa = (const float*)rp(bs, g.xa); p.xb = (const float*)rp(bs, g.xb); p.ca = g.ca; p.cb = g.cb;
                p.DHW = g.DHW; p.nslab = g.nslab; p.rows_per_slab = g.rows_per_slab; p.N = g.N; p.partial = (float*)rp(bs, g.partial);
                hipLaunchKernelGGL(gn_stats_f32_kernel, dim3(g.nslab, g.N), dim3(256), 0, s, p);
                break; }
            case OP_GN_APPLY32: {
                const GnRec& g = o.gn;
                if (g.nrb_a || g.nslab) {
                    Gn32FusedParams q{}; q.xa = (const float*)rp(bs, g.xa); q.xb = (const float*)rp(bs, g.xb); q.ca = g.ca; q.cb = g.cb;
                    q.DHW = g.DHW; q.N = g.N; q.silu = g.silu; q.groups = g.groups; q.rows_per_block = g.rows_per_block; q.eps = g.eps;
                    q.gamma = (const float*)rp(bs, g.gamma); q.beta = (const float*)rp(bs, g.beta);
                    if (g.nrb_a) {
                        q.sa = (const float*)rp(bs, g.stats_a); q.sb = (const float*)rp(bs, g.stats_b); q.nrb_a = g.nrb_a; q.nrb_b = g.nrb_b; q.nslab = 1;
                    } else { q.partial = (const float*)rp(bs, g.partial); q.nslab = g.nslab; }
                    if (g.out_hl) q.out_hl = (bf16_t*)rp(bs, g.out); else q.out = (float*)rp(bs, g.out);
                    hipLaunchKernelGGL(gn32_fold_apply_kernel, dim3(g.chunks, (g.ca + g.cb + 63) / 64, g.N), dim3(256), 0, s, q);
                } else {
                    Gn32Params p{}; p.xa = (const float*)rp(bs, g.xa); p.xb = (const float*)rp(bs, g.xb); p.ca = g.ca; p.cb = g.cb;
                    p.DHW = g.DHW; p.N = g.N; p.silu = g.silu; p.ab = (const float*)rp(bs, g.ab); p.out = (float*)rp(bs, g.out);
                    hipLaunchKernelGGL(gn_apply_f32_kernel, dim3(grid_for((long)g.N * g.DHW * ((g.ca + g.cb) / 4), 256, 4096)), dim3(256), 0, s, p);
                }
                break; }
            case OP_ATTN32: {
                Attn32Params p = attn_params<Attn32Params>(o.at, bs); p.x3 = o.at.x3;
                HIP_TRY(launch_attn_f32(p, s));
                break; }
            case OP_GEMV: case OP_GEMV32: {
                const LinRec& l = o.lin;
                const char* w = rp(bs, l.w); const float* bias = (const float*)rp(bs, l.bias); const float* x = (const float*)rp(bs, l.x);
                if (o.kind == OP_GEMV32 && !w) return fail(LDM_ERR_NOT_LOADED, "fp32 precision: the fp32 weight arena is empty");
                launch_gemv(w, o.kind == OP_GEMV32, bias, x, (float*)rp(bs, l.y), l.B, l.I, l.O, l.x_stride, l.y_stride, l.silu, s);
                break; }
            case OP_TAP: {
                const LayoutRec& l = o.lay;
                float* dst = (float*)rp(bs, l.dst); const float* src = (const float*)rp(bs, l.b);
                const long total = (long)l.N * l.c_real * l.DHW;
                if (dst) {
                    if (l.esz == 4) hipLaunchKernelGGL(tap_export_kernel<float>, dim3(grid_for(total)), dim3(256), 0, s, (const float*)rp(bs, l.a), dst, l.N, l.c_real, l.c_stored, l.DHW);
                    else hipLaunchKernelGGL(tap_export_kernel<bf16_t>, dim3(grid_for(total)), dim3(256), 0, s, (const bf16_t*)rp(bs, l.a), dst, l.N, l.c_real, l.c_stored, l.DHW);
                }
                if (src && l.mode == 2) {
                    launch_pack2(src, l.c_real, nullptr, 0, rp(bs, l.a), l.N, l.c_stored, l.DHW, l.esz == 4, s);
                }
                break; }
            case OP_FIN_GN: {
                const ConvRec& c = o.cv;
                FinGnParams q{}; q.f = finalize_params(conv_params(o, bs));
                q.gamma = (const float*)rp(bs, c.gamma); q.beta = (const float*)rp(bs, c.beta); q.y = (bf16_t*)rp(bs, c.gn_out);
                q.groups = c.gn_groups; q.silu = c.gn_silu; q.lg = c.gn_lg; q.eps = c.gn_eps;
                HIP_TRY(launch_fin_gn(q, c.N, wt_stores(), s));
                break; }
            case OP_CONV: case OP_FINALIZE: {
// ... 264 lines not shown
}
static void pack32_device(ldm_model* m, const ParamDesc& d, const float* src, hipStream_t s) {
    if (d.kind == PK_VEC_F32) return;
    float* dst = (float*)(m->arena32 + 2 * d.dst_off);
    const bool lin = d.kind == PK_LINEAR_W;
    const int taps = lin ? 1 : d.k * d.k * d.k, cin_s = lin ? d.cin : d.cin_s, cout_pad = lin ? d.cout : d.cout_pad, row_off = lin ? 0 : d.row_off;
    const long total = (long)taps * d.cout * cin_s;
    hipLaunchKernelGGL(param_pack_f32_kernel, dim3(grid_for(total, 256, 8192)), dim3(256), 0, s, src, dst, taps, d.cout, d.cin, cin_s, cout_pad, row_off);
}

int ldm_model_load_param(ldm_model* m, const char* name, const float* src, size_t numel) {
    if (!m || !name || !src) return fail(LDM_ERR_BAD_ARG, "null argument");
    auto it = m->pindex.find(name);
    if (it == m->pindex.end()) return fail(LDM_ERR_BAD_ARG, "unknown parameter '%s'", name);
    ParamDesc& d = m->params[it->second];
    size_t expect = 1; for (auto s : d.shape) expect *= (size_t)s;
    if (expect != numel) return fail(LDM_ERR_BAD_ARG, "parameter '%s': expected %zu elements, got %zu", name, expect, numel);
    LDM_TRY(ensure_arena(m));
    if (d.kind == PK_VEC_F32) {
        HIP_TRY(hipMemcpy(m->arena + d.dst_off, src, numel * 4, hipMemcpyHostToDevice));
    } else if (d.kind == PK_LINEAR_W) {
        std::vector<uint16_t> tmp(numel);
        for (size_t k = 0; k < numel; ++k) tmp[k] = host_f2bf(src[k]);
        HIP_TRY(hipMemcpy(m->arena + d.dst_off, tmp.data(), numel * 2, hipMemcpyHostToDevice));
    } else {
        const int taps = d.k * d.k * d.k;
        std::vector<uint16_t> tmp((size_t)d.cout * d.cin_s);
        for (int t = 0; t < taps; ++t) {
            std::fill(tmp.begin(), tmp.end(), (uint16_t)0);
            for (int co = 0; co < d.cout; ++co)
                for (int ci = 0; ci < d.cin; ++ci)
                    tmp[(size_t)co * d.cin_s + ci] = host_f2bf(src[((size_t)co * d.cin + ci) * taps + t]);
            char* dst = m->arena + d.dst_off + ((size_t)t * d.cout_pad + d.row_off) * d.cin_s * 2;
            HIP_TRY(hipMemcpy(dst, tmp.data(), tmp.size() * 2, hipMemcpyHostToDevice));
        }
    }
    if (m->precision == 1 && d.kind != PK_VEC_F32) {
        LDM_TRY(ensure_arena32(m));
        if (d.kind == PK_LINEAR_W) {
            HIP_TRY(hipMemcpy(m->arena32 + 2 * d.dst_off, src, numel * 4, hipMemcpyHostToDevice));
        } else {
            const int taps = d.k * d.k * d.k;
            std::vector<float> tmp((size_t)d.cout * d.cin_s);
            for (int t = 0; t < taps; ++t) {
                std::fill(tmp.begin(), tmp.end(), 0.f);
                for (int co = 0; co < d.cout; ++co)
                    for (int ci = 0; ci < d.cin; ++ci)
                        tmp[(size_t)co * d.cin_s + ci] = src[((size_t)co * d.cin + ci) * taps + t];
                char* dst = m->arena32 + 2 * (d.dst_off + ((size_t)t * d.cout_pad + d.row_off) * d.cin_s * 2);
                HIP_TRY(hipMemcpy(dst, tmp.data(), tmp.size() * 4, hipMemcpyHostToDevice));
            }
        }
    }
    if (!d.loaded) { d.loaded = true; m->loaded_count++; }
    m->derived_dirty = true; m->temb_tab_valid = false;
    return 0;
}

static int ensure_derived(ldm_model* m, hipStream_t s) {
    if (!m->derived_dirty) return 0;
    for (const auto& iw : m->im2col_ws)
        launch_im2col_weights((const bf16_t*)(m->arena + iw.w_off), (bf16_t*)(m->arena + iw.wi_off), iw.cout_pad, iw.cin_s, iw.cin, iw.Kp, s);
    for (const auto& pw : m->phase_ws)
        launch_phase_weights((const bf16_t*)(m->arena + pw.w_off), (bf16_t*)(m->arena + pw.wp_off), pw.cout_pad, pw.cin_s, s);
    if (m->precision == 1 && m->arena32)
        for (const auto& xw : m->x3p_ws)
            launch_x3_phase_weights((const float*)(m->arena32 + 2 * xw.w_off), (bf16_t*)(m->arena32 + 2 * m->arena_bytes + xw.x3p_off), xw.cout_pad, xw.cin_s, s);
    if (m->precision == 1 && m->arena32)
        for (const auto& xw : m->x3_ws)
            launch_x3_weights((const float*)(m->arena32 + 2 * xw.w_off), (bf16_t*)(m->arena32 + 2 * m->arena_bytes + xw.x3_off), xw.rows, xw.cin_s, s);
    HIP_TRY(hipGetLastError());
    m->derived_dirty = false;
    return 0;
}

static int get_plan(ldm_model* m, const char* kind, int B, int D, int H, int W, std::shared_ptr<Plan>* out, int tap_mode = 0) {
    if (B < 1 || D < 1 || H < 1 || W < 1 || D > 255 * 8 || H > 255 * 8 || W > 255 * 8) return fail(LDM_ERR_BAD_ARG, "bad shape");
    const bool train = kind[0] == 't';
    const bool hp = m->precision == 1;
    char key[96]; snprintf(key, sizeof key, "%s:%d:%d:%d:%d:p%d:t%d", kind, B, D, H, W, hp ? 1 : 0, tap_mode);
    auto it = m->plans.find(key);
    if (it != m->plans.end()) { *out = it->second; return 0; }
    std::shared_ptr<Plan> p(new Plan());
    if (m->type == 0) LDM_TRY(unet_build(m, B, D, H, W, p.get(), train, hp, tap_mode, strcmp(kind, "unet_tab") == 0 || strcmp(kind, "unet_cfg_tab") == 0,
                                     strncmp(kind, "unet_cfg", 8) == 0));
    else if (train) LDM_TRY(vae_build_train(m, B, D, H, W, p.get(), hp));
    else if (kind[0] == 'e') LDM_TRY(vae_build_encode(m, B, D, H, W, p.get(), hp, tap_mode));
    else LDM_TRY(vae_build_decode(m, B, D, H, W, p.get(), hp, tap_mode));
    m->plans[key] = p; *out = p;
    return 0;
}

static int check_ready(ldm_model* m, const void* ws, size_t ws_bytes, const Plan& p) {
    if (m->loaded_count != (int)m->params.size()) {
        for (auto& d : m->params) if (!d.loaded)
            return fail(LDM_ERR_NOT_LOADED, "parameter '%s' (and %d others) not uploaded", d.name.c_str(),
                        (int)m->params.size() - m->loaded_count - 1);
    }
    if (!ws || ws_bytes < p.ws_bytes) return fail(LDM_ERR_WORKSPACE, "workspace too small: need %zu bytes, got %zu", p.ws_bytes, ws_bytes);
    if (((uintptr_t)ws) & 255) return fail(LDM_ERR_BAD_ARG, "workspace must be 256-byte aligned");
    if (p.wt_tab.ready() || p.exp_tab.ready() || p.cs_tab.ready()) return fail(LDM_ERR_HIP, "descriptor table upload failed");
    return 0;
}

static int ready_plan(ldm_model* m, const char* kind, int B, int D, int H, int W, const void* ws, size_t ws_bytes, std::shared_ptr<Plan>* out,
                      int tap_mode = 0) {
    LDM_TRY(get_plan(m, kind, B, D, H, W, out, tap_mode));
    return check_ready(m, ws, ws_bytes, **out);
}
static Bases model_bases(const ldm_model* m, void* workspace) {
    Bases bs{}; bs.p[BASE_WS] = (char*)workspace; bs.p[BASE_W] = m->arena; bs.p[BASE_W32] = m->arena32;
    return bs;
}

size_t ldm_unet_workspace_bytes(ldm_model* m, int B, int D, int H, int W) {
    if (!m || m->type != 0) { fail(LDM_ERR_BAD_ARG, "not a UNet handle"); return 0; }
    std::shared_ptr<Plan> p; if (get_plan(m, "unet", B, D, H, W, &p)) return 0;
    return p->ws_bytes;
}

static std::atomic<uint64_t> g_sampler_uid{0};
struct ldm_sampler;
struct ldm_likelihood {
    ldm_sampler* rows = nullptr; std::vector<float> host; int n_steps = 0, pred = 0, clip = 1, next = 0;
    unsigned seed_lo = 0, seed_hi = 0; float half_bin = 0.f; const float* noise = nullptr;
};
struct ldm_sampler {
    float* coef = nullptr; SamplerState* st = nullptr; int n_steps = 0, kind = 0, clip = 1, pred = PRED_EPSILON; unsigned seed_lo = 0, seed_hi = 0;
    uint64_t uid = ++g_sampler_uid;
    float* state = nullptr; int64_t state_n = 0;
    std::vector<float> ts;
    int repaint = 0, known_batch = 0; const float* known = nullptr; const float* keep = nullptr; int64_t rp_per_sample = 0, rp_dhw = 0;
};
enum { SAMPLER_DDPM = 0, SAMPLER_DDIM = 1, SAMPLER_PNDM = 2, SAMPLER_RFLOW = 3, SAMPLER_DPM = 4 };
static bool sampler_multistep(const ldm_sampler* sp) { return sp->kind == SAMPLER_PNDM || sp->kind == SAMPLER_DPM; }
static const char* sampler_multistep_name(const ldm_sampler* sp) { return sp->kind == SAMPLER_DPM ? "DPM-Solver++" : "PNDM"; }
static int sampler_row_len(const ldm_sampler* sp) {
    return sp->repaint ? (int)REPAINT_ROW : sp->kind == SAMPLER_PNDM ? (int)PNDM_ROW : sp->kind == SAMPLER_DPM ? (int)DPM_ROW : 8;
}
static int repaint_check(const ldm_sampler* sp, int64_t n, int64_t samples) {
    if (!sp->repaint) return 0;
    if (!sp->known || !sp->keep) return fail(LDM_ERR_BAD_ARG, "repaint sampler without a known latent and keep mask: call ldm_sampler_bind_known first");
    if (samples < 1 || n != samples * sp->rp_per_sample)
        return fail(LDM_ERR_BAD_ARG, "repaint sampler: bound for samples of %lld elements, the step has %lld elements on %lld samples",
                    (long long)sp->rp_per_sample, (long long)n, (long long)samples);
    if (sp->known_batch != 1 && sp->known_batch != samples)
        return fail(LDM_ERR_BAD_ARG, "repaint sampler: known_batch must be 1 or the step's %lld samples, got %d", (long long)samples, sp->known_batch);
    return 0;
}
static int repaint_launch(ldm_sampler* sp, const float* m, float* x, float* x0_out, int64_t n, float* tbuf, int B, hipStream_t s,
                          const WinGeom* geom, float* xw, int C);
static int dpm_launch(ldm_sampler* sp, const float* m, float* x, float* x0_out, int64_t n, float* tbuf, int B, hipStream_t s,
                      const WinGeom* geom, float* xw, int C);
static std::atomic<uint64_t> g_grid_uid{0};
struct ldm_window_grid {
    int dims[3] = {0, 0, 0}, roi[3] = {0, 0, 0}, n[3] = {0, 0, 0};
    char* dev = nullptr;
    WinGeom geom{};
    uint64_t uid = ++g_grid_uid;
    int64_t n_windows() const { return (int64_t)n[0] * n[1] * n[2]; }
    int64_t roi_vox() const { return (int64_t)roi[0] * roi[1] * roi[2]; }
    int64_t vox() const { return (int64_t)dims[0] * dims[1] * dims[2]; }
};
extern "C++" template <bool SAMPLE = true, class Launch>
static void with_pred(int pred, Launch&& launch) {
    if constexpr (SAMPLE) if (pred == PRED_SAMPLE) return launch(std::integral_constant<int, PRED_SAMPLE>{});
    if (pred == PRED_V) return launch(std::integral_constant<int, PRED_V>{});
    launch(std::integral_constant<int, PRED_EPSILON>{});
// ... 53 lines not shown
    hipError_t e = hipMemcpyAsync(d_t, sp->ts.data(), (size_t)n * 4, hipMemcpyHostToDevice, s);
    if (e == hipSuccess) {
        const LinW& l0 = m->lins.at("time_embed.0"); const LinW& l2 = m->lins.at("time_embed.2");
        launch_sinusoid((const float*)d_t, d_sin, n, c0, s);
        auto gemv = [&](size_t w_off, size_t b_off, const float* xin, float* y, int I, int O, int silu) {
            launch_gemv(hp ? m->arena32 + 2 * w_off : m->arena + w_off, hp, (const float*)(m->arena + b_off), xin, y, n, I, O, I, O, silu, s);
        };
        gemv(l0.w_off, l0.b_off, d_sin, d_e1, c0, temb, 0);
        gemv(l2.w_off, l2.b_off, d_e1, d_e2, temb, temb, 1);
        gemv(m->tproj_w_off, m->tproj_b_off, d_e2, m->temb_tab, temb, rows, 1);
        e = hipGetLastError();
        if (e == hipSuccess) e = hipStreamSynchronize(s);
    }
    (void)hipFree(tmp);
    if (e != hipSuccess) return fail(LDM_ERR_HIP, "time-embedding table: %s", hipGetErrorString(e));
    m->temb_tab_ts = sp->ts; m->temb_tab_prec = m->precision; m->temb_tab_valid = true;
    return 0;
}

extern "C++" template <class RunAll>
static int graph_run(ldm_model* m, const ldm_model::GraphKey& key, hipStream_t stream, RunAll&& run_all) {
    ldm_model::GraphEntry* ge = nullptr;
    for (size_t k = 0; k < m->graphs.size();) {
        const auto& g = m->graphs[k].key;
        if ((key.ptr[6] && g.ptr[6] == key.ptr[6] && g.sampler_uid != key.sampler_uid) ||
            (key.grid && g.grid == key.grid && g.grid_uid != key.grid_uid)) {
            if (m->graphs[k].exec) (void)hipGraphExecDestroy(m->graphs[k].exec);
            m->graphs.erase(m->graphs.begin() + k);
        } else ++k;
    }
    for (auto& g : m->graphs) if (!memcmp(&g.key, &key, sizeof key)) { ge = &g; break; }
    if (!ge) {
        if (m->graphs.size() >= 16) {
            if (m->graphs.front().exec) (void)hipGraphExecDestroy(m->graphs.front().exec);
            m->graphs.erase(m->graphs.begin());
        }
        m->graphs.emplace_back(); ge = &m->graphs.back();
        memcpy(&ge->key, &key, sizeof key); ge->seen = 0; ge->exec = nullptr;
    }
    if (ge->exec) { HIP_TRY(hipGraphLaunch(ge->exec, stream)); return 0; }
    if (ge->seen++ == 0) return run_all(stream);
    hipGraph_t graph = nullptr;
    if (!m->cap_stream) HIP_TRY(hipStreamCreateWithFlags(&m->cap_stream, hipStreamNonBlocking));
    HIP_TRY(hipStreamBeginCapture(m->cap_stream, hipStreamCaptureModeThreadLocal));
    const int rc = run_all(m->cap_stream);
    const hipError_t ec = hipStreamEndCapture(m->cap_stream, &graph);
    if (rc) { if (graph) (void)hipGraphDestroy(graph); return rc; }
    if (ec != hipSuccess || !graph) return fail(LDM_ERR_HIP, "stream capture failed: %s", hipGetErrorString(ec));
    HIP_TRY(hipGraphInstantiate(&ge->exec, graph, nullptr, nullptr, 0));
    (void)hipGraphDestroy(graph);
    HIP_TRY(hipGraphLaunch(ge->exec, stream));
    return 0;
}

struct Guide { float w, fill; };
struct LikStep { const ldm_likelihood* lk; const float* x0; float* kl_map; float* terms; float* total; void* scratch; };
static int likelihood_tail(const LikStep& ls, float* x_t, const float* m_out, float* tbuf, int B, int64_t per_sample, hipStream_t s);
struct StepArgs {
    const float* x; int x_channels; const float* cond; int cond_channels; float* tbuf; float* out;
    int B; int64_t total; int D, H, W;
    void* workspace; size_t workspace_bytes; void* stream;
    ldm_sampler* sp; float* latent; const Guide* guide; const LikStep* lik; const ldm_window_grid* grid;
};
static int unet_step(ldm_model* m, StepArgs a) {
    if (!m || m->type != 0) return fail(LDM_ERR_BAD_ARG, "not a UNet handle");
    if (!a.x || !a.tbuf || !a.out) return fail(LDM_ERR_BAD_ARG, "null tensor argument");
    if (!a.cond) a.cond_channels = 0;
    const Guide* const guide = a.guide; ldm_sampler* const sp = a.sp; const ldm_window_grid* const grid = a.grid;
    const int gm = guide ? 2 : 1;
    const bool tab = sp != nullptr && temb_table_enabled() && m->tproj_rows % 4 == 0;
    const char* kind = guide ? (tab ? "unet_cfg_tab" : "unet_cfg") : tab ? "unet_tab" : "unet";
    const int ragged = a.B > 0 ? (int)(a.total % a.B) : 0;
    std::shared_ptr<Plan> p, p2;
    LDM_TRY(ready_plan(m, kind, gm * a.B, a.D, a.H, a.W, a.workspace, a.workspace_bytes, &p));
    if (ragged) LDM_TRY(ready_plan(m, kind, gm * ragged, a.D, a.H, a.W, a.workspace, a.workspace_bytes, &p2));
    const int64_t per_out = (int64_t)m->ucfg.out_channels * a.D * a.H * a.W, per_x = (int64_t)a.x_channels * a.D * a.H * a.W;
    float* pair = nullptr;
    if (guide && grid) {
        const size_t pair_off = rup_sz(std::max(p->ws_bytes, p2 ? p2->ws_bytes : (size_t)0), 256), need = pair_off + (size_t)2 * a.B * per_out * 4;
        if (a.workspace_bytes < need)
            return fail(LDM_ERR_WORKSPACE, "workspace too small for the guided windows: need %zu bytes, got %zu", need, a.workspace_bytes);
        pair = (float*)((char*)a.workspace + pair_off);
    }
    if (tab) LDM_TRY(ensure_temb_table(m, sp, (hipStream_t)a.stream));
    Bases bs = model_bases(m, a.workspace);
    bs.p[BASE_IO2] = (char*)a.tbuf;
    if (tab) { bs.p[BASE_TTAB] = (char*)m->temb_tab; bs.p[BASE_SST] = (char*)sp->st; bs.sampler_steps = sp->n_steps; }
    if (guide) bs.guide_fill = guide->fill;
    const int rt[2] = {a.x_channels, a.cond_channels};
    LDM_TRY(ensure_derived(m, (hipStream_t)a.stream));
    auto run_all = [&](hipStream_t s) -> int {
        for (int64_t b0 = 0; b0 < a.total; b0 += a.B) {
            const bool last = b0 + a.B > a.total;
            float* dst = a.out + b0 * per_out;
            float* raw = pair ? pair : dst;
            Bases cb = bs;
            cb.p[BASE_IO0] = (char*)(a.x + b0 * per_x);
            cb.p[BASE_IO1] = a.cond ? (char*)(a.cond + b0 * a.cond_channels * a.D * a.H * a.W) : nullptr;
            cb.p[BASE_IO3] = (char*)raw;
            LDM_TRY(run_plan(last ? *p2 : *p, cb, rt, s));
            if (guide) {
                const int64_t ne = (last ? ragged : a.B) * per_out;
                guided_combine_launch(raw, raw + ne, guide->w, dst, ne, s);
            }
        }
        if (a.lik) return likelihood_tail(*a.lik, a.latent, a.out, a.tbuf, a.B, per_out, s);
        if (!sp) return 0;
        if (!grid) return sampler_launch(sp, a.out, a.latent, nullptr, a.total * per_out, a.tbuf, gm * a.B, s);
        return sampler_launch(sp, a.out, a.latent, nullptr, grid->vox() * a.x_channels, a.tbuf, gm * a.B, s, &grid->geom, const_cast<float*>(a.x), a.x_channels);
    };
    if (!m->graph_mode || g_prof.on || g_plan_trace.on) return run_all((hipStream_t)a.stream);
    ldm_model::GraphKey key; memset(&key, 0, sizeof key);
    key.plan[0] = p.get(); key.plan[1] = p2.get();
    const void* ptr[8] = {a.x, a.cond, a.tbuf, a.out, a.workspace, a.stream, sp, a.latent};
    memcpy(key.ptr, ptr, sizeof ptr); key.rt[0] = rt[0]; key.rt[1] = rt[1]; key.chunk = a.B;
    if (sp) { key.sampler_uid = sp->uid; key.sampler_state = sp->state; }
    if (grid) { key.grid = grid; key.grid_uid = grid->uid; }
    if (guide) { key.guide[0] = guide->w; key.guide[1] = guide->fill; }
    if (a.lik) { const void* lp[6] = {a.lik->x0, a.lik->lk->noise, a.lik->kl_map, a.lik->terms, a.lik->total, a.lik->scratch}; memcpy(key.lik, lp, sizeof lp); }
    return graph_run(m, key, (hipStream_t)a.stream, run_all);
}
int ldm_unet_forward(ldm_model* m, const float* x, int x_channels, const float* cond, int cond_channels,
                     const float* timesteps, float* out, int B, int D, int H, int W,
                     void* workspace, size_t workspace_bytes, void* stream) {
    return unet_step(m, {x, x_channels, cond, cond_channels, (float*)timesteps, out, B, B, D, H, W, workspace, workspace_bytes, stream});
}

static int sampler_alloc(const float* coef_host, int row_len, int n_steps, std::unique_ptr<ldm_sampler>* out) {
    std::unique_ptr<ldm_sampler> sp(new ldm_sampler());
    const size_t bytes = (size_t)n_steps * row_len * 4;
    HIP_TRY(hipMalloc((void**)&sp->coef, bytes));
    HIP_TRY(hipMemcpy(sp->coef, coef_host, bytes, hipMemcpyHostToDevice));
    HIP_TRY(hipMalloc((void**)&sp->st, 256));
    HIP_TRY(hipMemset(sp->st, 0, 256));
    HIP_TRY(hipDeviceSynchronize());
    sp->n_steps = n_steps;
    sp->ts.resize(n_steps); for (int k = 0; k < n_steps; ++k) sp->ts[k] = coef_host[(size_t)k * row_len + 5];
    *out = std::move(sp);
    return 0;
}
int ldm_sampler_create(const float* coef_host, int n_steps, int kind, int pred, int clip, uint64_t seed, ldm_sampler** out) {
    if (!coef_host || n_steps < 1 || kind < 0 || kind > 1 || !out) return fail(LDM_ERR_BAD_ARG, "bad argument");
    if (pred < PRED_EPSILON || pred > PRED_V) return fail(LDM_ERR_BAD_ARG, "unknown prediction type %d (0 epsilon, 1 sample, 2 v_prediction)", pred);
    std::unique_ptr<ldm_sampler> sp; LDM_TRY(sampler_alloc(coef_host, 8, n_steps, &sp));
    sp->kind = kind; sp->pred = pred; sp->clip = clip ? 1 : 0; sp->seed_lo = (unsigned)seed; sp->seed_hi = (unsigned)(seed >> 32);
    *out = sp.release();
    return 0;
}
int ldm_sampler_create_pndm(const float* coef_host, int n_steps, int pred, ldm_sampler** out) {
    if (!coef_host || n_steps < 1 || !out) return fail(LDM_ERR_BAD_ARG, "bad argument");
    if (pred != PRED_EPSILON && pred != PRED_V) return fail(LDM_ERR_BAD_ARG, "PNDM takes prediction type 0 (epsilon) or 2 (v_prediction), got %d", pred);
    static_assert(PNDM_ROW == LDM_PNDM_ROW, "row stride of the header");
    int pushes = 0; bool saved = false, acc = false;
    for (int k = 0; k < n_steps; ++k) {
        const float* r = coef_host + (size_t)k * PNDM_ROW;
        const PndmCoef c = pndm_coef(r);
        if (r[4] != (float)c.flags || c.flags < 0 || c.flags >= 32 || r[12] != (float)c.head || c.head != pushes)
            return fail(LDM_ERR_BAD_ARG, "PNDM row %d: bad flags / head (head must count the pushes of the rows before it)", k);
        if ((c.flags & PNDM_ACC_SET) && (c.flags & PNDM_ACC_ADD)) return fail(LDM_ERR_BAD_ARG, "PNDM row %d: accumulator both set and added to", k);
        const int depth = c.w3 != 0.f ? 3 : c.w2 != 0.f ? 2 : c.w1 != 0.f ? 1 : 0;
        if (depth > pushes) return fail(LDM_ERR_BAD_ARG, "PNDM row %d reads %d history slots, %d written so far", k, depth, pushes);
        if ((c.flags & PNDM_USE_SAVED) && !saved) return fail(LDM_ERR_BAD_ARG, "PNDM row %d reads the saved sample before any row saved one", k);
        if ((c.wacc != 0.f || (c.flags & PNDM_ACC_ADD)) && !acc) return fail(LDM_ERR_BAD_ARG, "PNDM row %d reads the accumulator before any row set it", k);
        if (c.flags & PNDM_PUSH) ++pushes;
        if (c.flags & PNDM_SAVE) saved = true;
        if (c.flags & PNDM_ACC_SET) acc = true;
    }
    std::unique_ptr<ldm_sampler> sp; LDM_TRY(sampler_alloc(coef_host, PNDM_ROW, n_steps, &sp));
    sp->kind = SAMPLER_PNDM; sp->pred = pred; sp->clip = 0;
    *out = sp.release();
    return 0;
}
int ldm_sampler_create_rflow(const float* coef_host, int n_steps, ldm_sampler** out) {
    if (!coef_host || n_steps < 1 || !out) return fail(LDM_ERR_BAD_ARG, "bad argument");
    for (int k = 0; k < n_steps; ++k) {
        const float* r = coef_host + (size_t)k * 8;
        if (!std::isfinite(r[0]) || !std::isfinite(r[1]) || !std::isfinite(r[5])) return fail(LDM_ERR_BAD_ARG, "rectified-flow row %d is not finite", k);
    }
    std::unique_ptr<ldm_sampler> sp; LDM_TRY(sampler_alloc(coef_host, 8, n_steps, &sp));
    sp->kind = SAMPLER_RFLOW; sp->pred = PRED_EPSILON; sp->clip = 0;
    *out = sp.release();
    return 0;
}
size_t ldm_sampler_state_bytes(const ldm_sampler* sp, int64_t n) {
    if (!sp || n < 0) { fail(LDM_ERR_BAD_ARG, "bad argument"); return 0; }
    return sp->kind == SAMPLER_PNDM ? (size_t)n * 6 * sizeof(float) : sp->kind == SAMPLER_DPM ? (size_t)n * sizeof(float) : 0;
}
int ldm_sampler_bind_state(ldm_sampler* sp, void* state, size_t bytes, int64_t n) {
    if (!sp || !state || n < 0) return fail(LDM_ERR_BAD_ARG, "bad argument");
    if (!sampler_multistep(sp)) return fail(LDM_ERR_BAD_ARG, "only a PNDM or DPM-Solver++ sampler takes a state buffer");
// ... 2356 lines not shown
    sp->uid = ++g_sampler_uid;
    return 0;
}
int ldm_sampler_repaint_noise(const ldm_sampler* sp, int which, int row, float* out, int64_t n, void* stream) {
    if (!sp || !out || n < 0 || row < 0 || which < 0 || which > 1) return fail(LDM_ERR_BAD_ARG, "bad argument");
    if (!sp->repaint) return fail(LDM_ERR_BAD_ARG, "not a repaint sampler");
    hipLaunchKernelGGL(repaint_noise_kernel<0>, dim3(grid_for((n + 3) / 4, 256, 1024)), dim3(256), 0, (hipStream_t)stream, out, (long)n,
                       (unsigned)row, which ? REPAINT_JUMP_STREAM_TAG : REPAINT_KNOWN_STREAM_TAG, sp->seed_lo, sp->seed_hi);
    HIP_TRY(hipGetLastError());
    return 0;
}
int ldm_repaint_merge(const float* x, const float* known, int known_batch, const float* keep, const float* z_known, const float* z_jump,
                      float* out, int B, int64_t per_sample, int64_t dhw, const float* coef4_host, int jump, void* stream) {
    if (!x || !known || !keep || !out || !coef4_host) return fail(LDM_ERR_BAD_ARG, "null argument");
    if (B < 1 || B > 65535) return fail(LDM_ERR_BAD_ARG, "B must be in 1 .. 65535, got %d", B);
    if (dhw < 1 || per_sample < dhw || per_sample % dhw || per_sample > ((int64_t)1 << 33))
        return fail(LDM_ERR_BAD_ARG, "per_sample (%lld) must be a multiple of dhw (%lld) in 1 .. 2^33", (long long)per_sample, (long long)dhw);
    if (known_batch != 1 && known_batch != B) return fail(LDM_ERR_BAD_ARG, "known_batch must be 1 or B = %d, got %d", B, known_batch);
    if (jump != 0 && jump != 1) return fail(LDM_ERR_BAD_ARG, "jump must be 0 or 1, got %d", jump);
    LDM_TRY(repaint_check_coef(coef4_host, (float)jump, 0));
    if (coef4_host[1] != 0.f && !z_known) return fail(LDM_ERR_BAD_ARG, "ks != 0 needs z_known");
    if (jump && coef4_host[3] != 0.f && !z_jump) return fail(LDM_ERR_BAD_ARG, "a jump with js != 0 needs z_jump");
    RepaintMergeParams p{};
    p.x = x; p.known = known; p.keep = keep; p.zk = coef4_host[1] != 0.f ? z_known : nullptr; p.zj = jump && coef4_host[3] != 0.f ? z_jump : nullptr;
    p.out = out; p.n = (long)(B * per_sample); p.per_sample = (long)per_sample; p.dhw = (long)dhw; p.known_batch = known_batch;
    p.c = RepaintCoef{coef4_host[0], coef4_host[1], coef4_host[2], coef4_host[3], jump};
    hipLaunchKernelGGL(repaint_merge_kernel<0>, dim3(grid_for((p.n + 3) / 4, 256, 1024)), dim3(256), 0, (hipStream_t)stream, p);
    HIP_TRY(hipGetLastError());
    return 0;
}

static int dpm_launch(ldm_sampler* sp, const float* m, float* x, float* x0_out, int64_t n, float* tbuf, int B, hipStream_t s,
                      const WinGeom* geom, float* xw, int C) {
    StepParams p = step_params(sp); p.m = m; p.x = x; p.x0_out = x0_out; p.n = (long)n; p.tbuf = tbuf; p.B = B; p.xw = xw; p.C = C;
    const dim3 grid(grid_for((n + 3) / 4, 256, 1024));
    with_pred(sp->pred, [&](auto P) {
        if (!geom) hipLaunchKernelGGL(dpm_sampler_step_kernel<P()>, grid, dim3(256), 0, s, p);
        else hipLaunchKernelGGL(dpm_window_step_kernel<P()>, grid, dim3(256), 0, s, *geom, p);
    });
    return 0;
}
static int dpm_check_row(const float* r, int k) {
    for (int j = 0; j < DPM_ROW; ++j) if (!std::isfinite(r[j])) return fail(LDM_ERR_BAD_ARG, "DPM-Solver++ row %d is not finite", k);
    const DpmCoef c = dpm_coef(r);
    if (r[4] != (float)c.flags || c.flags < 0 || c.flags >= 8) return fail(LDM_ERR_BAD_ARG, "DPM-Solver++ row %d: bad flags", k);
    if (c.cz < 0.f) return fail(LDM_ERR_BAD_ARG, "DPM-Solver++ row %d: cz is a standard deviation and may not be negative", k);
    if (((c.flags & DPM_DRAWS) != 0) != (c.cz != 0.f)) return fail(LDM_ERR_BAD_ARG, "DPM-Solver++ row %d: the DRAWS flag must be set exactly when cz != 0", k);
    if (!(c.flags & DPM_HAS_PREV) && c.c1 != 0.f) return fail(LDM_ERR_BAD_ARG, "DPM-Solver++ row %d: c1 != 0 without the HAS_PREV flag", k);
    if ((c.flags & DPM_CLIP) && !(c.clip_min <= c.clip_max)) return fail(LDM_ERR_BAD_ARG, "DPM-Solver++ row %d: clip_min above clip_max", k);
    return 0;
}
int ldm_sampler_create_dpm(const float* coef_host, int n_steps, int pred, uint64_t seed, ldm_sampler** out) {
    if (!coef_host || n_steps < 1 || !out) return fail(LDM_ERR_BAD_ARG, "bad argument");
    if (pred < PRED_EPSILON || pred > PRED_V) return fail(LDM_ERR_BAD_ARG, "unknown prediction type %d (0 epsilon, 1 sample, 2 v_prediction)", pred);
    static_assert(DPM_ROW == LDM_DPM_ROW && DPM_HAS_PREV == LDM_DPM_HAS_PREV && DPM_DRAWS == LDM_DPM_DRAWS && DPM_CLIP == LDM_DPM_CLIP,
                  "row layout of the header");
    for (int k = 0; k < n_steps; ++k) LDM_TRY(dpm_check_row(coef_host + (size_t)k * DPM_ROW, k));
    if ((int)coef_host[4] & DPM_HAS_PREV) return fail(LDM_ERR_BAD_ARG, "DPM-Solver++ row 0 reads the previous x0_hat before any row wrote one");
    std::unique_ptr<ldm_sampler> sp; LDM_TRY(sampler_alloc(coef_host, DPM_ROW, n_steps, &sp));
    sp->kind = SAMPLER_DPM; sp->pred = pred; sp->clip = 0; sp->seed_lo = (unsigned)seed; sp->seed_hi = (unsigned)(seed >> 32);
    *out = sp.release();
    return 0;
}
int ldm_dpm_step(const float* m, const float* x, const float* prev_x0_in, const float* z, float* prev_x0_out, float* x_out, float* x0_out,
                 int64_t n, int pred, const float* row, void* stream) {
    if (!m || !x || !x_out || !row || n < 0 || x_out == x || x_out == m) return fail(LDM_ERR_BAD_ARG, "bad argument");
    if (pred < PRED_EPSILON || pred > PRED_V) return fail(LDM_ERR_BAD_ARG, "unknown prediction type %d (0 epsilon, 1 sample, 2 v_prediction)", pred);
    LDM_TRY(dpm_check_row(row, 0));
    const DpmCoef c = dpm_coef(row);
    const bool has_prev = (c.flags & DPM_HAS_PREV) != 0, draws = (c.flags & DPM_DRAWS) != 0;
    if ((has_prev && !prev_x0_in) || (draws && !z)) return fail(LDM_ERR_BAD_ARG, "DPM-Solver++ step: the row reads state or noise that was passed as NULL");
    const float* pi = has_prev ? prev_x0_in : nullptr; const float* zz = draws ? z : nullptr;
    if (x_out == pi || x_out == zz || (prev_x0_out && (prev_x0_out == x_out || prev_x0_out == m || prev_x0_out == x)) ||
        (x0_out && (x0_out == x_out || x0_out == m || x0_out == x || x0_out == pi)))
        return fail(LDM_ERR_BAD_ARG, "DPM-Solver++ step: an output aliases an input it may not");
    hipStream_t s = (hipStream_t)stream;
    const dim3 g(grid_for((n + 3) / 4, 256, 1024));
    with_pred(pred, [&](auto P) { hipLaunchKernelGGL(dpm_step_kernel<P()>, g, dim3(256), 0, s, m, x, pi, zz, prev_x0_out, x_out, x0_out, (long)n, c); });
    HIP_TRY(hipGetLastError());
    return 0;
}

}
```

### 3d-latent-diffusion-model_amd/profiling.py

```python
from __future__ import annotations

import collections
import os
from typing import Dict, List, Optional

from . import _lib

KINDS = ("PACK CONV FINALIZE GN_STATS GN_FINALIZE GN_PREP GN_APPLY ATTN SINUSOID GEMV VAE_HEADS GN_FUSED WT WT_BATCH WGRAD EXPORT "
         "EXPORT_BATCH COLSUM GNB ATTN_BWD ADD SUMPOOL LIN_DX LIN_DW VAE_HEADS_BWD GEMM_LIGHT COLSUM_BATCH IM2COL "
         "PACK32 CONV32 FIN32 GN_STATS32 GN_APPLY32 ATTN32 GEMV32 TAP BUCKET BUCKET_JOIN UPS_SPLIT32 CONV_THIN FIN_GN GEMM_LIGHT32 CONV_BLOCK TEMB_ROW").split()


def summarize(path: str) -> Dict[str, List[float]]:
    out: Dict[str, List[float]] = collections.defaultdict(lambda: [0, 0.0])
    with open(path) as fh:
        for ln in fh:
            parts = ln.rstrip("\n").split(",", 4)
            if len(parts) < 4:
                continue
            k = int(parts[2])
            name = KINDS[k] if 0 <= k < len(KINDS) else f"KIND{k}"
            out[name][0] += 1
            out[name][1] += float(parts[3])
    return dict(out)


class PlanProfiler:
    def __init__(self, out_dir: str = "./profiler_logs", wait: int = 1, warmup: int = 1, active: int = 3, repeat: int = 2,
                 verbose: bool = True):
        self.out_dir, self.wait, self.warmup, self.active, self.repeat, self.verbose = out_dir, wait, warmup, active, repeat, verbose
        os.makedirs(out_dir, exist_ok=True)
        self.step_idx = 0
        self.paths: List[str] = []
        self._current: Optional[str] = None
        self._apply()

    def _phase(self):
        cycle_len = self.wait + self.warmup + self.active
        cycle, pos = divmod(self.step_idx, cycle_len)
        if cycle >= self.repeat:
            return None
        return cycle if pos >= self.wait + self.warmup else None

    def _apply(self):
        cycle = self._phase()
        want = None if cycle is None else os.path.join(self.out_dir, f"plan_trace_cycle{cycle}.csv")
        if want == self._current:
            return
        L = _lib.lib()
        if self._current is not None and want != self._current:
            _lib.check(L.ldm_set_plan_trace(None))
            self._report(self._current)
        if want is not None:
            if os.path.exists(want):
                os.remove(want)
            _lib.check(L.ldm_set_plan_trace(want.encode()))
            self.paths.append(want)
        self._current = want

    def _report(self, path: str):
        if not self.verbose or not os.path.exists(path):
            return
        groups = summarize(path)
        total = sum(v[1] for v in groups.values()) or 1.0
        print(f"[profile] {path}: {total / max(1, self.active) / 1e3:.3f} ms of launch-plan ops per traced step")
        for name, (n, us) in sorted(groups.items(), key=lambda kv: -kv[1][1])[:12]:
            print(f"[profile]   {name:14s} {us / self.active:10.1f} us/step  {100 * us / total:5.1f} %  ({n // max(1, self.active)} ops/step)")

    def step(self):
        self.step_idx += 1
        self._apply()

    def stop(self):
        if self._current is not None:
            _lib.check(_lib.lib().ldm_set_plan_trace(None))
            self._report(self._current)
            self._current = None
```

### include/ldm3d.h

```cpp
#ifndef LDM3D_H
#define LDM3D_H
#include <stddef.h>
#include <stdint.h>

#ifdef __cplusplus
extern "C" {
#endif

#define LDM_MAX_LEVELS 8
#define LDM_ABI_VERSION 1

typedef enum {
    LDM_OK = 0,
    LDM_ERR_BAD_ARG = -1,
    LDM_ERR_UNSUPPORTED = -2,
    LDM_ERR_HIP = -3,
    LDM_ERR_NOT_LOADED = -4,
    LDM_ERR_WORKSPACE = -5,
    LDM_ERR_RCCL = -6
} ldm_status;

typedef struct {
    int spatial_dims;
    int in_channels, out_channels;
// ... 263 lines not shown
                            int N, int Din, int Hin, int Win, int ksize, int stride, int pad, int ups, int ksplit, void* stream);
int ldm_op_attention_f32(const float* qkv, float* out, float* lse, int B, int N, int C, int head_dim, int x3, void* stream);
int ldm_op_attention_bwd_f32(const float* qkv, const float* o, const float* d_o, const float* lse, float* delta_scratch, float* dqkv,
                             int B, int N, int C, int head_dim, void* stream);
int ldm_op_group_norm_bwd2_f32(const float* dy, const float* xa, int ca, const float* xb, int cb, const float* gamma, const float* beta,
                               int groups, float eps, int act, const float* acc_a, const float* acc_b, float* dxa, float* dxb,
                               float* dgamma, float* dbeta, int N, int DHW, void* scratch, size_t scratch_bytes, void* stream);
int ldm_op_upsample_bwd_f32(const float* dy, float* dx, int N, int D, int H, int W, int C, void* stream);
size_t ldm_op_group_norm_bwd_saved_scratch_bytes(int N, int C, int DHW, int groups);
int ldm_op_group_norm_bwd_fold_chunks(int N, int C, int groups, int DHW);
int ldm_op_group_norm_bwd_saved(const void* dy, const void* xa, int ca, const void* xb, int cb, const float* ab, const float* mr,
                                const float* gamma, int groups, int act, const void* acc_a, const void* acc_b, void* dxa, void* dxb,
                                float* dgamma, float* dbeta, float* cs, int N, int DHW, int form, void* scratch, size_t scratch_bytes,
                                void* stream);
size_t ldm_op_colsum_finalize_ws_bytes(const int64_t* desc, int k);
int ldm_op_colsum_finalize(const float* partial, float* out, const int64_t* desc, int k, int batched, void* desc_ws, size_t desc_ws_bytes,
                           void* stream);
size_t ldm_op_grad_export_ws_bytes(const int64_t* desc, int k);
int ldm_op_grad_export(const float* src, float* dst, const int64_t* desc, int k, int batched, void* desc_ws, size_t desc_ws_bytes, void* stream);
size_t ldm_op_weight_flip_transpose_batched_ws_bytes(const int64_t* desc, int k);
int ldm_op_weight_flip_transpose_batched(const void* w, void* wt, const int64_t* desc, int k, void* desc_ws, size_t desc_ws_bytes, void* stream);
int ldm_op_linear_bwd_nz(int O);
int ldm_op_linear_bwd(const void* W, const float* dy, const float* x_pre, float* dx, float* dW, float* db, int B, int I, int O, int dy_stride,
                      int x_stride, int silu_in, float* part, size_t part_bytes, void* stream);
int ldm_op_upsample_bwd(const void* dy, void* dx, int N, int D, int H, int W, int C, void* stream);
int ldm_op_add_bf16(const void* a, const void* b, void* out, int64_t n, void* stream);
int ldm_op_vae_heads(const float* ml, const float* eps, float* mu, float* sigma, float* z, int N, int L, int DHW, void* stream);
int ldm_op_vae_heads_bwd(const void* dz, int Ls, const float* ml, const float* z, const float* g_mu, const float* g_sigma, void* dy,
                         int N, int L, int Cs, int DHW, int fp32, void* stream);
size_t ldm_op_conv3d_fin_gn_scratch_bytes(int N, int D, int H, int W, int cout_pad, int splitk);
int ldm_op_conv3d_fin_gn(const void* x, int cin, const void* w, const float* bias, const float* temb, int temb_stride, const void* residual,
                         const float* gamma, const float* beta, int groups, float eps, int silu, void* conv_out, void* gn_out,
                         int N, int D, int H, int W, int cout, int cout_pad, int wgn, int splitk, void* scratch, size_t scratch_bytes,
                         void* stream);
size_t ldm_op_conv3d_gn_scratch_bytes(int N, int D, int H, int W, int cout_pad, int splitk);
int ldm_op_conv3d_gn(const void* x, int cin, const void* w, const float* bias, const float* gamma, const float* beta, int groups, float eps,
                     int silu, void* conv_out, void* gn_out, int N, int D, int H, int W, int cout, int cout_pad, int wgn, int splitk,
                     void* scratch, size_t scratch_bytes, void* stream);
size_t ldm_op_group_norm_scratch_bytes(int N, int C, int DHW);
int ldm_op_group_norm(const void* xa, int ca, const void* xb, int cb, const float* gamma, const float* beta,
                      int groups, float eps, int silu, void* out, int N, int DHW, void* scratch, size_t scratch_bytes,
                      void* stream);
int ldm_op_attention(const void* qkv, void* out, int B, int N, int C, void* stream);
int ldm_op_attention_hd(const void* qkv, void* out, float* lse, int B, int N, int C, int head_dim, void* stream);
int ldm_op_attention_bwd_hd(const void* qkv, const void* o, const void* d_o, const float* lse, float* delta_scratch, void* dqkv,
                            int B, int N, int C, int head_dim, void* stream);
int ldm_op_attention_train(const void* qkv, void* out, float* lse, int B, int N, int C, void* stream);
int ldm_op_attention_bwd(const void* qkv, const void* o, const void* d_o, const float* lse, float* delta_scratch, void* dqkv,
                         int B, int N, int C, void* stream);

int ldm_profile_start(int wgm, int wgn, int bk, int max_launches);
int ldm_profile_detail(double* flops, double* ms, int max);
int ldm_profile_stop(double out[5]);
int ldm_set_plan_trace(const char* path);
int ldm_debug_kstamps(unsigned long long* out, int max_entries, int reset);
int ldm_model_plan_conv_cfgs(ldm_model* m, const char* kind, int B, int D, int H, int W, int* cfgs, int max_convs);
int ldm_model_plan_launches(ldm_model* m, const char* kind, int B, int D, int H, int W);

typedef struct ldm_comm ldm_comm;
int ldm_comm_unique_id(char id[128]);
int ldm_comm_init(int rank, int world, const char id[128], ldm_comm** out);
typedef int (*ldm_allreduce_fn)(void* user, void* buf, int64_t count, int dtype, int op, void* stream);
int ldm_comm_init_custom(int rank, int world, ldm_allreduce_fn fn, void* user, ldm_comm** out);
int ldm_comm_allreduce(ldm_comm* c, void* buf, int64_t count, int dtype, int op, void* stream);
int ldm_comm_broadcast(ldm_comm* c, void* buf, int64_t count, int dtype, int root, void* stream);
int ldm_comm_barrier(ldm_comm* c, void* stream);
void ldm_comm_destroy(ldm_comm* c);
int ldm_comm_rank(const ldm_comm* c);
int ldm_comm_world(const ldm_comm* c);
int ldm_model_set_grad_sync(ldm_model* m, ldm_comm* comm);
int ldm_model_grad_sync_trace(ldm_model* m, double* issue_ms, double* done_ms, int64_t* elems, int max);
int ldm_model_set_grad_wire(ldm_model* m, int dtype);
int ldm_model_grad_sync_pending(const ldm_model* m);
int ldm_comm_stats(const ldm_comm* c, int64_t out[4]);
int ldm_comm_is_rccl(const ldm_comm* c);
int ldm_comm_rccl_version(void);
int ldm_model_grad_schedule(ldm_model* m, int B, int D, int H, int W, int* kind, int64_t* lo, int64_t* n, int* op, int max);

int ldm_op_conv3d_thin(const void* x_bf16_ndhwc, int cin, const void* w_packed, const float* bias, float* out_f32_ncdhw, int N, int D, int H, int W,
                       int cout_real, int cout_pad, void* stream);
size_t ldm_op_conv3d_thin_f32_ws_bytes(int cin, int N, int D, int H, int W, int cout_pad);
int ldm_op_conv3d_thin_f32(const float* x_f32_ndhwc, int cin, const float* w_packed, const float* bias, float* out_f32_ncdhw, int N, int D, int H,
                           int W, int cout_real, int cout_pad, void* ws, size_t ws_bytes, void* stream);
int ldm_op_timestep_embedding(const float* t, float* out, int B, int dim, void* stream);
int ldm_op_gemv(const void* w, int fp32_weights, const float* bias, const float* x, float* y, int B, int I, int O, int x_stride, int y_stride,
                int silu_in, void* stream);
int ldm_op_pack2(const float* x, int cx, const float* cond, int cc, void* out, int N, int Cs, int64_t DHW, int fp32_out, int guided_B, float fill,
                 void* stream);
int ldm_op_pack_im2col(const float* x, int cx, const float* cond, int cc, void* out, int N, int D, int H, int W, int Kp, int guided_B, float fill,
                       void* stream);
int ldm_op_phase_weights(const void* w3, void* wp, int cout_pad, int cin_s, void* stream);
int ldm_op_im2col_weights(const void* w3, void* w2, int cout_pad, int cin_s, int cin, int Kp, void* stream);
int ldm_op_x3_weights(const float* w, void* out, int64_t rows, int cin, void* stream);
int ldm_op_x3_phase_weights(const float* w3, void* wp, int cout_pad, int cin, void* stream);
int ldm_op_split_f32(const float* x, void* out, int N, int C, int D, int H, int W, int up, void* stream);

#ifdef __cplusplus
}
#endif
#endif
```

Measured before the change: 526.4.

## Add tiled MFMA kernel for the UNet output conv with optional fused sampler step

Adds a dedicated 3x3x3 conv kernel for the final thin-output conv (at most 4 output channels). Each block owns a 2x4x8 voxel tile, stages a halo of input channels and the weights in LDS with double-buffered register prefetch, and runs bf16 MFMA. It is aimed at the thin conv path, which uses the machine poorly on this small latent. An optional mode (off by default via LDM_OUT_STEP) also fuses the DDPM/DDIM sampler update into the epilogue to save a launch. The kernel only replaces the thin conv when the tile count falls between a minimum and the CU count, so coverage depends on shape.

```diff
diff --git a/3d-latent-diffusion-model_amd/_lib.py b/3d-latent-diffusion-model_amd/_lib.py
--- a/3d-latent-diffusion-model_amd/_lib.py
+++ b/3d-latent-diffusion-model_amd/_lib.py
@@ -245,6 +245,8 @@
     "ldm_op_conv3d_thin": (C.c_int, [_P, C.c_int, _P, _P, _P] + [C.c_int] * 6 + [_P]),
     "ldm_op_conv3d_thin_f32_ws_bytes": (C.c_size_t, [C.c_int] * 6),
     "ldm_op_conv3d_thin_f32": (C.c_int, [_P, C.c_int, _P, _P, _P] + [C.c_int] * 6 + [_P, C.c_size_t, _P]),
+    "ldm_op_conv3d_out": (C.c_int, [_P, C.c_int, _P, _P, _P] + [C.c_int] * 6 + [_P]),
+    "ldm_op_conv3d_out_step": (C.c_int, [_P, C.c_int, _P, _P, _P] + [C.c_int] * 6 + [_P, _P, _P, C.c_int, _P]),
     "ldm_op_timestep_embedding": (C.c_int, [_P, _P, C.c_int, C.c_int, _P]),
     "ldm_op_gemv": (C.c_int, [_P, C.c_int, _P, _P, _P] + [C.c_int] * 6 + [_P]),
     "ldm_op_pack2": (C.c_int, [_P, C.c_int, _P, C.c_int, _P, C.c_int, C.c_int, C.c_int64, C.c_int, C.c_int, C.c_float, _P]),
diff --git a/3d-latent-diffusion-model_amd/csrc/conv_out.h b/3d-latent-diffusion-model_amd/csrc/conv_out.h
--- /dev/null
+++ b/3d-latent-diffusion-model_amd/csrc/conv_out.h
@@ -0,0 +1,187 @@
+#pragma once
+#include "common.h"
+#include "norm_elem.h"
+
+struct OutParams {
+    const bf16_t* x; const bf16_t* w;
+    const float* bias; float* out;
+    int N, D, H, W, Cin, CoutPad, CoutReal;
+    int td, th, tw;
+    StepParams step;
+};
+
+constexpr int OUT_TD = 2, OUT_TH = 4, OUT_TW = 8;
+constexpr int OUT_HD = OUT_TD + 2, OUT_HH = OUT_TH + 2, OUT_HW = OUT_TW + 2;
+constexpr int OUT_HV = OUT_HD * OUT_HH * OUT_HW;
+constexpr int OUT_CK = 32, OUT_RB = OUT_CK * 2, OUT_NC = OUT_RB / 16;
+constexpr int OUT_LDS_X = OUT_HV * OUT_RB, OUT_LDS_W = 27 * 4 * OUT_RB;
+constexpr int OUT_GC = 2, OUT_GS = OUT_GC * OUT_NC, OUT_GR = 256 / OUT_GS;
+constexpr int OUT_PLANE = OUT_LDS_X + OUT_LDS_W + 64;
+constexpr int OUT_LDS = OUT_GC * OUT_PLANE;
+constexpr int OUT_NX = (OUT_HV + OUT_GR - 1) / OUT_GR, OUT_NW = (27 * 4 + OUT_GR - 1) / OUT_GR;
+constexpr int OUT_VOX = OUT_TD * OUT_TH * OUT_TW;
+static_assert(256 % OUT_GS == 0, "a thread keeps its slot over the items of a group");
+
+static inline long conv_out_tiles(int N, int D, int H, int W) {
+    return (long)N * ((D + OUT_TD - 1) / OUT_TD) * ((H + OUT_TH - 1) / OUT_TH) * ((W + OUT_TW - 1) / OUT_TW);
+}
+
+__device__ __forceinline__ int out_swz(int hv) { return (hv >> 1) & (OUT_NC - 1); }
+
+struct OutRegs { u32x4 x[OUT_NX]; u32x4 w[OUT_NW]; };
+
+template <bool FUSE, int PRED>
+__global__ __launch_bounds__(256) void conv3_out_kernel(const OutParams p) {
+#if defined(__HIP_DEVICE_COMPILE__)
+    __shared__ __attribute__((aligned(16))) char smem[OUT_LDS];
+    const int tid = threadIdx.x, lane = tid & 63, wave = tid >> 6, fr = lane & 15, fg = lane >> 4;
+    int k = 0;
+    if constexpr (FUSE) k = p.step.st->k;
+    int b = xcd_remap((int)blockIdx.x, (int)gridDim.x);
+    const int bw = b % p.tw; b /= p.tw; const int bh = b % p.th; b /= p.th; const int bd = b % p.td; const int n = b / p.td;
+    const int d0 = bd * OUT_TD, h0 = bh * OUT_TH, w0 = bw * OUT_TW;
+    const int ci = fr < 4 ? fr : fr < 12 ? fr - 4 : fr - 8;
+    const int hl = (wave & 1) * 2 + (ci >> 2), wl = (ci & 1) + ((ci >> 1) & 1) * 4 + ((fr >= 4 && fr < 12) ? 2 : 0), dl = wave >> 1;
+    const int hv0 = (dl * OUT_HH + hl) * OUT_HW + wl;
+
+    const int s16 = tid & (OUT_GS - 1), hr = tid / OUT_GS;
+    const int pl = (s16 >> 2) * OUT_PLANE, sub = s16 & (OUT_NC - 1);
+    const u32x4 zero = {0u, 0u, 0u, 0u};
+    auto load_group = [&](OutRegs& r, int g) {
+        const int c = g * OUT_GC * OUT_CK + s16 * 8;
+        const bool con = c < p.Cin;
+#pragma unroll
+        for (int i = 0; i < OUT_NX; ++i) {
+            const int hv = hr + OUT_GR * i;
+            const int wx = hv % OUT_HW, q = hv / OUT_HW, hy = q % OUT_HH, dz = q / OUT_HH;
+            const int gd = d0 - 1 + dz, gh = h0 - 1 + hy, gw = w0 - 1 + wx;
+            r.x[i] = zero;
+            if (con && hv < OUT_HV && (unsigned)gd < (unsigned)p.D && (unsigned)gh < (unsigned)p.H && (unsigned)gw < (unsigned)p.W)
+                r.x[i] = *reinterpret_cast<const u32x4*>(p.x + ((((size_t)n * p.D + gd) * p.H + gh) * p.W + gw) * p.Cin + c);
+        }
+#pragma unroll
+        for (int i = 0; i < OUT_NW; ++i) {
+            const int tr = hr + OUT_GR * i;
+            r.w[i] = zero;
+            if (con && tr < 27 * 4 && (tr & 3) < p.CoutReal)
+                r.w[i] = *reinterpret_cast<const u32x4*>(p.w + ((size_t)(tr >> 2) * p.CoutPad + (tr & 3)) * p.Cin + c);
+        }
+    };
+    auto store_group = [&](const OutRegs& r, int g) {
+        if (g * OUT_GC * OUT_CK + s16 * 8 >= p.Cin) return;
+#pragma unroll
+        for (int i = 0; i < OUT_NX; ++i) {
+            const int hv = hr + OUT_GR * i;
+            if (hv < OUT_HV) *reinterpret_cast<u32x4*>(smem + pl + hv * OUT_RB + ((sub ^ out_swz(hv)) << 4)) = r.x[i];
+        }
+#pragma unroll
+        for (int i = 0; i < OUT_NW; ++i) {
+            const int tr = hr + OUT_GR * i;
+            if (tr < 27 * 4 && (tr & 3) < p.CoutReal)
+                *reinterpret_cast<u32x4*>(smem + pl + OUT_LDS_X + tr * OUT_RB + ((sub ^ (tr & 3)) << 4)) = r.w[i];
+        }
+    };
+    f32x4 acc = {0.f, 0.f, 0.f, 0.f};
+    const int nchunk = p.Cin / OUT_CK, ngroup = (nchunk + OUT_GC - 1) / OUT_GC;
+    const unsigned wmask = fr < p.CoutReal ? 0xffffffffu : 0u;
+    auto taps_group = [&](int g) {
+        const int nck = nchunk - g * OUT_GC < OUT_GC ? nchunk - g * OUT_GC : OUT_GC;
+#pragma unroll 1
+        for (int c = 0; c < nck; ++c) {
+            const char* buf = smem + c * OUT_PLANE;
+            const int wrow = fr & 3;
+            const char* wbase = buf + OUT_LDS_X + wrow * OUT_RB + ((fg ^ wrow) << 4);
+            u32x4 fw[3][3], fx[3][3];
+            auto rd = [&](int bt) {
+#pragma unroll
+                for (int t = 0; t < 3; ++t) {
+                    const int tap = bt * 3 + t, kd = tap / 9, kh = (tap / 3) % 3, kw = tap % 3;
+                    const int hv = hv0 + (kd * OUT_HH + kh) * OUT_HW + kw;
+                    fw[bt % 3][t] = *reinterpret_cast<const u32x4*>(wbase + tap * 4 * OUT_RB);
+                    fx[bt % 3][t] = *reinterpret_cast<const u32x4*>(buf + hv * OUT_RB + ((fg ^ out_swz(hv)) << 4));
+                }
+            };
+            rd(0); rd(1);
+#pragma unroll
+            for (int bt = 0; bt < 9; ++bt) {
+                if (bt + 2 < 9) rd(bt + 2);
+                __builtin_amdgcn_sched_barrier(0);
+#pragma unroll
+                for (int t = 0; t < 3; ++t) {
+                    u32x4 wr = fw[bt % 3][t];
+                    wr.x &= wmask; wr.y &= wmask; wr.z &= wmask; wr.w &= wmask;
+                    acc = __builtin_amdgcn_mfma_f32_16x16x32_bf16(*reinterpret_cast<const bf16x8*>(&wr), *reinterpret_cast<const bf16x8*>(&fx[bt % 3][t]), acc, 0, 0, 0);
+                }
+                __builtin_amdgcn_sched_barrier(0);
+            }
+        }
+    };
+
+    OutRegs ra, rb;
+    load_group(ra, 0);
+    if (ngroup > 1) load_group(rb, 1);
+
+    const StepParams& sp = p.step;
+    const int qr = tid >> 4, qj = tid & 15;
+    const int qd = d0 + (qj >> 3), qh = h0 + ((qj >> 1) & 3), qw = w0 + (qj & 1) * 4;
+    const size_t dhw = (size_t)p.D * p.H * p.W;
+    const bool quad = FUSE && tid < 64 && qr < p.CoutReal && qd < p.D && qh < p.H && qw < p.W;
+    const long i0 = (long)(((size_t)n * p.CoutReal + qr) * dhw + ((size_t)qd * p.H + qh) * p.W + qw);
+    float4 xq = make_float4(0.f, 0.f, 0.f, 0.f), zq = xq;
+    SamplerCoef sc{};
+    bool live = false;
+    if constexpr (FUSE) {
+        sc = sampler_coef<PRED>(sp.coef, k, sp.n_steps);
+        live = k < sp.n_steps;
+        if (quad && live) {
+            xq = *reinterpret_cast<const float4*>(sp.x + i0);
+            if (sc.sigma != 0.f) zq = sampler_normal4((unsigned long long)(i0 >> 2), (unsigned)k, sp.seed_lo, sp.seed_hi);
+        }
+    }
+
+    for (int g = 0; g < ngroup; g += 2) {
+        if (g) __syncthreads();
+        store_group(ra, g);
+        if (g + 2 < ngroup) load_group(ra, g + 2);
+        __syncthreads();
+        taps_group(g);
+        if (g + 1 < ngroup) {
+            __syncthreads();
+            store_group(rb, g + 1);
+            if (g + 3 < ngroup) load_group(rb, g + 3);
+            __syncthreads();
+            taps_group(g + 1);
+        }
+    }
+    __syncthreads();
+    float* se = reinterpret_cast<float*>(smem);
+    if (fg == 0) {
+        const int v = (dl * OUT_TH + hl) * OUT_TW + wl;
+#pragma unroll
+        for (int r = 0; r < 4; ++r)
+            if (r < p.CoutReal) se[r * OUT_VOX + v] = acc[r] + (p.bias ? p.bias[r] : 0.f);
+    }
+    __syncthreads();
+    if constexpr (!FUSE) {
+        const int r = tid >> 6, v = tid & 63;
+        const int gd = d0 + v / (OUT_TH * OUT_TW), gh = h0 + (v / OUT_TW) % OUT_TH, gw = w0 + v % OUT_TW;
+        if (r < p.CoutReal && gd < p.D && gh < p.H && gw < p.W)
+            p.out[((size_t)n * p.CoutReal + r) * dhw + ((size_t)gd * p.H + gh) * p.W + gw] = se[r * OUT_VOX + v];
+    } else {
+        if (quad) {
+            const float4 m = *reinterpret_cast<const float4*>(se + qr * OUT_VOX + (qj >> 1) * OUT_TW + (qj & 1) * 4);
+            *reinterpret_cast<float4*>(p.out + i0) = m;
+            if (live) {
+                float x0;
+                float4 xn;
+                xn.x = sampler_update<PRED>(sc, sp.kind, sp.clip, xq.x, m.x, zq.x, &x0);
+                xn.y = sampler_update<PRED>(sc, sp.kind, sp.clip, xq.y, m.y, zq.y, &x0);
+                xn.z = sampler_update<PRED>(sc, sp.kind, sp.clip, xq.z, m.z, zq.z, &x0);
+                xn.w = sampler_update<PRED>(sc, sp.kind, sp.clip, xq.w, m.w, zq.w, &x0);
+                *reinterpret_cast<float4*>(sp.x + i0) = xn;
+            }
+        }
+        sampler_advance(sp.st, sp.coef, sp.n_steps, k, sp.tbuf, sp.B, StepRule<PRED, STEP_DDPM>::stride);
+    }
+#endif
+}
diff --git a/3d-latent-diffusion-model_amd/csrc/ldm3d.hip b/3d-latent-diffusion-model_amd/csrc/ldm3d.hip
--- a/3d-latent-diffusion-model_amd/csrc/ldm3d.hip
+++ b/3d-latent-diffusion-model_amd/csrc/ldm3d.hip
@@ -157,7 +157,8 @@
               OP_FIN_GN,
               OP_GEMM_LIGHT32,
               OP_CONV_BLOCK,
-              OP_TEMB_ROW };
+              OP_TEMB_ROW,
+              OP_CONV_OUT };
 
 struct ConvCfg { int wgm, wgn, bk, splitk; int halo = 0, mtps = 0, qps = 0; int slab_lg = 0; int cube = 0; int th = 0, big = 0; int plane = 0; int wg = 0; };
 
@@ -174,6 +175,7 @@
     bool ep32_ndhwc, ep32_ncdhw;
     Ref bias, bias2, temb, residual; int temb_stride;
     Ref out; int f32_out;
+    bool step;
     Ref partial, stats;
     int stats_nrb, stats_rows;
     Ref gamma, beta, gn_out; int gn_groups, gn_silu, gn_lg; float gn_eps;
@@ -531,6 +533,7 @@
     }
     bool train = false, recording = false;
     bool guided = false;
+    bool out_conv = false, out_step = false;
 
     struct ConvArgs {
         Act xa, xb;
@@ -687,6 +690,12 @@
         Op op{}; op.kind = OP_CONV_THIN;
         ConvRec& c = op.cv; c = conv_rec(a, 3, 1, 1, M, cout_real); conv_epilogue(c, a, Act());
         c.xa = ws_ref(a.xa.off); c.ca = x3 ? 2 * a.xa.C : a.xa.C; c.x3 = x3; c.w = w;
+        plan->ops.push_back(op);
+    }
+    void emit_out(const ConvArgs& a, long M, Ref w, int cout_real) {
+        Op op{}; op.kind = OP_CONV_OUT;
+        ConvRec& c = op.cv; c = conv_rec(a, 3, 1, 1, M, cout_real); conv_epilogue(c, a, Act());
+        c.xa = ws_ref(a.xa.off); c.ca = a.xa.C; c.w = w; c.step = out_step;
         plan->ops.push_back(op);
     }
     Act emit_light(OpKind kind, const ConvArgs& a, long M, Ref w, int big, bool want_stats) {
@@ -896,6 +905,15 @@
                 record_conv(a, Act());
                 return Act();
             }
+            static const int out_thin = ldm_knob("LDM_OUT_THIN", 1);
+            static const long out_min = ldm_knob("LDM_OUT_THIN_MIN", 128L);
+            if (out_thin && thin && out_conv && !train && (long)N * ((a.Do + 1) / 2) * ((a.Ho + 3) / 4) * ((a.Wo + 7) / 8) >= out_min &&
+                (long)N * ((a.Do + 1) / 2) * ((a.Ho + 3) / 4) * ((a.Wo + 7) / 8) <= std::max((long)device_cus(), out_min) && a.f32_out && a.k == 3 && a.stride == 1 && a.pad == 1 && !a.ups && !a.exact && !a.xb.valid && !a.w1 &&
+                a.temb.base == BASE_NULL && !a.residual.valid && a.w_over.base == BASE_NULL && cr <= 4 && cin0 % 32 == 0 && cin0 <= 512 &&
+                a.xa.D == a.Do && a.xa.H == a.Ho && a.xa.W == a.Wo) {
+                emit_out(a, M, w_ref(w.w_off), cr);
+                return Act();
+            }
         }
         const bool phase = a.ups == 1 && !a.exact && a.k == 3 && a.stride == 1 && a.pad == 1 && !train && !a.xb.valid && !a.w1 &&
                            a.w_over.base == BASE_NULL && w.wp_off != 0 && phase_enabled() &&
@@ -1509,12 +1527,13 @@
 }
 
 static int unet_build(ldm_model* m, int B, int D, int H, int W, Plan* plan, bool train, bool hp = false, int tap_mode = 0, bool temb_table = false,
-                      bool guided = false) {
+                      bool guided = false, int out_mode = 0) {
     const ldm_unet_cfg& c = m->ucfg;
     const int L = c.num_levels; const int* ch = c.channels;
     const int temb = ch[0] * 4, G = c.norm_num_groups; const float eps = c.norm_eps;
     if (train && tap_mode) return fail(LDM_ERR_UNSUPPORTED, "debug taps are inference-only");
     Builder b; b.m = m; b.plan = plan; b.train = train; b.recording = train; b.hp = hp; b.tap_mode = tap_mode; b.guided = guided;
+    b.out_conv = out_mode >= 1 && !train; b.out_step = out_mode == 2 && !train;
     const size_t sin_off = b.pool.alloc((size_t)B * ch[0] * 4);
     const size_t e1_off = b.pool.alloc((size_t)B * temb * 4);
     const size_t e2_off = b.pool.alloc((size_t)B * temb * 4);
@@ -1870,7 +1889,8 @@
     return 0;
 }
 
-struct Bases { char* p[BASE_COUNT]; int sampler_steps; float guide_fill; };
+struct OutStep { StepParams p; int pred; };
+struct Bases { char* p[BASE_COUNT]; int sampler_steps; float guide_fill; const OutStep* out_step; };
 static inline char* rp(const Bases& b, const Ref& r) { return r.base == BASE_NULL ? nullptr : (b.p[r.base] ? b.p[r.base] + r.off : nullptr); }
 
 static int xcd_rows_mode() { static const int v = ldm_xknob("LDM_XCD_ROWS", 0); return v; }
@@ -2362,6 +2382,7 @@
 struct LaneCtx { GradSyncState* sync = nullptr; };
 static void guided_layout_launch(OpKind kind, const LayoutRec& l, const float* x, int cx, const float* cond, int cc, float fill, void* dst, hipStream_t s);
 static void guided_combine_launch(const float* u, const float* c, float w, float* out, int64_t n, hipStream_t s);
+static int conv_out_launch(const ConvRec& c, const Bases& bs, const OutStep* step, hipStream_t s);
 
 static int run_plan(const Plan& plan, const Bases& bs, const int* rt, hipStream_t s, size_t begin = 0, size_t end = (size_t)-1,
                     LaneCtx lanes = LaneCtx()) {
@@ -2393,6 +2414,7 @@
                         case OP_CONV32: case OP_FIN32: six(c.ca, c.cb, c.stats_nrb, c.stats_rows, c.N, c.Din); break;
                         case OP_CONV_THIN: six(c.N, c.Din, c.Hin, c.Win, c.x3 ? c.ca / 2 * 3 : c.ca, c.cout_pad); break;
                         case OP_CONV_BLOCK: six(c.N, c.Dout, c.Hout, c.Wout, c.ca, o.cc.th); break;
+                        case OP_CONV_OUT: six(c.N, c.Din, c.Hin, c.Win, c.ca, c.step); break;
                         case OP_GEMM_LIGHT: case OP_GEMM_LIGHT32: six(c.M, c.ca + c.cb, c.couts, c.cout_pad, o.cc.big, c.ca); break;
                         case OP_GN_STATS: case OP_GN_STATS32: six(g.ca, g.cb, g.DHW, g.nslab, g.rows_per_slab, g.N); break;
                         case OP_GN_FINALIZE: six(g.nslab, g.ca + g.cb, g.groups, g.DHW, g.N, 0); break;
@@ -2454,6 +2476,12 @@
                 if (c.x3) { q.x3_c = c.ca / 2; q.Cin = 3 * q.x3_c; } else q.Cin = c.ca;
                 if (!q.w) return fail(LDM_ERR_NOT_LOADED, "the weight arena is empty");
                 HIP_TRY(launch_conv_thin(q, s));
+                break; }
+            case OP_CONV_OUT: {
+                const ConvRec& c = o.cv;
+                if (c.step && !bs.out_step) return fail(LDM_ERR_BAD_ARG, "a step plan ran without a sampler");
+                if (g_prof.on) { g_prof.flops_all += 2.0 * (double)c.M * (double)c.cout_real * 27.0 * (double)c.ca; g_prof.launches_all++; }
+                LDM_TRY(conv_out_launch(c, bs, c.step ? bs.out_step : nullptr, s));
                 break; }
             case OP_CONV_BLOCK: {
                 const ConvRec& c = o.cv;
@@ -2884,8 +2912,9 @@
     auto it = m->plans.find(key);
     if (it != m->plans.end()) { *out = it->second; return 0; }
     std::shared_ptr<Plan> p(new Plan());
-    if (m->type == 0) LDM_TRY(unet_build(m, B, D, H, W, p.get(), train, hp, tap_mode, strcmp(kind, "unet_tab") == 0 || strcmp(kind, "unet_cfg_tab") == 0,
-                                     strncmp(kind, "unet_cfg", 8) == 0));
+    if (m->type == 0) LDM_TRY(unet_build(m, B, D, H, W, p.get(), train, hp, tap_mode, strcmp(kind, "unet_tab") == 0 || strcmp(kind, "unet_cfg_tab") == 0 ||
+                                     strcmp(kind, "unet_tab_step") == 0, strncmp(kind, "unet_cfg", 8) == 0,
+                                     strcmp(kind, "unet_tab_step") == 0 ? 2 : (strcmp(kind, "unet_tab") == 0 || strcmp(kind, "unet_cfg_tab") == 0) ? 1 : 0));
     else if (train) LDM_TRY(vae_build_train(m, B, D, H, W, p.get(), hp));
     else if (kind[0] == 'e') LDM_TRY(vae_build_encode(m, B, D, H, W, p.get(), hp, tap_mode));
     else LDM_TRY(vae_build_decode(m, B, D, H, W, p.get(), hp, tap_mode));
@@ -3105,8 +3134,19 @@
             return fail(LDM_ERR_WORKSPACE, "workspace too small for the guided windows: need %zu bytes, got %zu", need, a.workspace_bytes);
         pair = (float*)((char*)a.workspace + pair_off);
     }
+    OutStep fused_step{};
+    static const int out_step_knob = ldm_knob("LDM_OUT_STEP", 0);
+    const bool fuse = out_step_knob && sp && sp->kind <= SAMPLER_DDIM && !sp->repaint && !guide && !grid && !a.lik && !ragged && a.total == a.B &&
+                      a.x_channels == m->ucfg.out_channels && a.latent && a.W % 4 == 0 && (uintptr_t)a.out % 16 == 0 && (uintptr_t)a.latent % 16 == 0 &&
+                      !p->ops.empty() && p->ops.back().kind == OP_CONV_OUT;
+    if (fuse) {
+        LDM_TRY(ready_plan(m, "unet_tab_step", a.B, a.D, a.H, a.W, a.workspace, a.workspace_bytes, &p));
+        fused_step.p = step_params(sp); fused_step.pred = sp->pred;
+        fused_step.p.x = a.latent; fused_step.p.n = (long)(a.total * per_out); fused_step.p.tbuf = a.tbuf; fused_step.p.B = a.B;
+    }
     if (tab) LDM_TRY(ensure_temb_table(m, sp, (hipStream_t)a.stream));
     Bases bs = model_bases(m, a.workspace);
+    if (fuse) bs.out_step = &fused_step;
     bs.p[BASE_IO2] = (char*)a.tbuf;
     if (tab) { bs.p[BASE_TTAB] = (char*)m->temb_tab; bs.p[BASE_SST] = (char*)sp->st; bs.sampler_steps = sp->n_steps; }
     if (guide) bs.guide_fill = guide->fill;
@@ -3128,7 +3168,7 @@
             }
         }
         if (a.lik) return likelihood_tail(*a.lik, a.latent, a.out, a.tbuf, a.B, per_out, s);
-        if (!sp) return 0;
+        if (!sp || fuse) return 0;
         if (!grid) return sampler_launch(sp, a.out, a.latent, nullptr, a.total * per_out, a.tbuf, gm * a.B, s);
         return sampler_launch(sp, a.out, a.latent, nullptr, grid->vox() * a.x_channels, a.tbuf, gm * a.B, s, &grid->geom, const_cast<float*>(a.x), a.x_channels);
     };
@@ -5651,3 +5691,55 @@
 }
 
 }
+#include "conv_out.h"
+extern "C" {
+static int launch_conv_out(OutParams q, const OutStep* step, hipStream_t s) {
+    q.td = (q.D + OUT_TD - 1) / OUT_TD; q.th = (q.H + OUT_TH - 1) / OUT_TH; q.tw = (q.W + OUT_TW - 1) / OUT_TW;
+    if (!q.x || !q.w || !q.out) return fail(LDM_ERR_BAD_ARG, "null tensor argument");
+    if ((long)q.N * q.D * q.H * q.W * q.Cin >= (1L << 31)) return fail(LDM_ERR_UNSUPPORTED, "conv3_out_kernel addresses its input with 31-bit element offsets");
+    const dim3 grid((unsigned)conv_out_tiles(q.N, q.D, q.H, q.W));
+    if (!step) { hipLaunchKernelGGL((conv3_out_kernel<false, PRED_EPSILON>), grid, dim3(256), 0, s, q); return 0; }
+    if (q.W % 4 || (uintptr_t)q.out % 16 || !step->p.x || (uintptr_t)step->p.x % 16 || step->p.n != (long)q.N * q.CoutReal * q.D * q.H * q.W)
+        return fail(LDM_ERR_UNSUPPORTED, "the fused step needs W %% 4 == 0, a 16-byte aligned output and a 16-byte aligned latent of the output's shape");
+    q.step = step->p; q.step.m = q.out; q.step.x0_out = nullptr;
+    with_pred(step->pred, [&](auto P) { hipLaunchKernelGGL((conv3_out_kernel<true, P()>), grid, dim3(256), 0, s, q); });
+    return 0;
+}
+static int conv_out_launch(const ConvRec& c, const Bases& bs, const OutStep* step, hipStream_t s) {
+    OutParams q{}; q.x = (const bf16_t*)rp(bs, c.xa); q.w = (const bf16_t*)rp(bs, c.w); q.bias = (const float*)rp(bs, c.bias); q.out = (float*)rp(bs, c.out);
+    q.N = c.N; q.D = c.Din; q.H = c.Hin; q.W = c.Win; q.Cin = c.ca; q.CoutPad = c.cout_pad; q.CoutReal = c.cout_real;
+    if (!q.w) return fail(LDM_ERR_NOT_LOADED, "the weight arena is empty");
+    return launch_conv_out(q, step, s);
+}
+static int out_args_ok(const void* x, const void* w, const void* out, int cin, int N, int D, int H, int W, int cout_real, int cout_pad) {
+    if (!x || !w || !out) return fail(LDM_ERR_BAD_ARG, "null tensor argument");
+    if (N < 1 || D < 1 || H < 1 || W < 1 || (long)N * D * H * W >= (1L << 31)) return fail(LDM_ERR_BAD_ARG, "bad volume");
+    if (cin < 32 || cin % 32) return fail(LDM_ERR_BAD_ARG, "cin must be a positive multiple of 32, got %d", cin);
+    if (cout_real < 1 || cout_real > 4 || cout_pad < cout_real) return fail(LDM_ERR_BAD_ARG, "cout_real 1 .. 4 <= cout_pad, got %d / %d", cout_real, cout_pad);
+    if (cin > 512) return fail(LDM_ERR_UNSUPPORTED, "conv3_out_kernel is planned for at most 512 input channels, got %d", cin);
+    return 0;
+}
+int ldm_op_conv3d_out(const void* x, int cin, const void* w, const float* bias, float* out, int N, int D, int H, int W, int cout_real,
+                      int cout_pad, void* stream) {
+    LDM_TRY(out_args_ok(x, w, out, cin, N, D, H, W, cout_real, cout_pad));
+    OutParams q{}; q.x = (const bf16_t*)x; q.w = (const bf16_t*)w; q.bias = bias; q.out = out;
+    q.N = N; q.D = D; q.H = H; q.W = W; q.Cin = cin; q.CoutPad = cout_pad; q.CoutReal = cout_real;
+    LDM_TRY(launch_conv_out(q, nullptr, (hipStream_t)stream));
+    HIP_TRY(hipGetLastError());
+    return 0;
+}
+int ldm_op_conv3d_out_step(const void* x, int cin, const void* w, const float* bias, float* out, int N, int D, int H, int W, int cout_real,
+                           int cout_pad, ldm_sampler* sp, float* x_latent, float* tbuf, int B, void* stream) {
+    LDM_TRY(out_args_ok(x, w, out, cin, N, D, H, W, cout_real, cout_pad));
+    if (!sp || !x_latent || !tbuf || B < 1 || x_latent == out) return fail(LDM_ERR_BAD_ARG, "bad argument");
+    if (sp->kind > SAMPLER_DDIM || sp->repaint) return fail(LDM_ERR_UNSUPPORTED, "the fused out conv + step exists for DDPM / DDIM samplers only");
+    if (W % 4) return fail(LDM_ERR_UNSUPPORTED, "the fused out conv + step needs W %% 4 == 0, got %d", W);
+    OutParams q{}; q.x = (const bf16_t*)x; q.w = (const bf16_t*)w; q.bias = bias; q.out = out;
+    q.N = N; q.D = D; q.H = H; q.W = W; q.Cin = cin; q.CoutPad = cout_pad; q.CoutReal = cout_real;
+    OutStep st{step_params(sp), sp->pred}; st.p.x = x_latent; st.p.n = (long)N * cout_real * D * H * W; st.p.tbuf = tbuf; st.p.B = B;
+    LDM_TRY(launch_conv_out(q, &st, (hipStream_t)stream));
+    HIP_TRY(hipGetLastError());
+    return 0;
+}
+
+}
diff --git a/3d-latent-diffusion-model_amd/profiling.py b/3d-latent-diffusion-model_amd/profiling.py
--- a/3d-latent-diffusion-model_amd/profiling.py
+++ b/3d-latent-diffusion-model_amd/profiling.py
@@ -8,7 +8,7 @@
 
 KINDS = ("PACK CONV FINALIZE GN_STATS GN_FINALIZE GN_PREP GN_APPLY ATTN SINUSOID GEMV VAE_HEADS GN_FUSED WT WT_BATCH WGRAD EXPORT "
          "EXPORT_BATCH COLSUM GNB ATTN_BWD ADD SUMPOOL LIN_DX LIN_DW VAE_HEADS_BWD GEMM_LIGHT COLSUM_BATCH IM2COL "
-         "PACK32 CONV32 FIN32 GN_STATS32 GN_APPLY32 ATTN32 GEMV32 TAP BUCKET BUCKET_JOIN UPS_SPLIT32 CONV_THIN FIN_GN GEMM_LIGHT32 CONV_BLOCK TEMB_ROW").split()
+         "PACK32 CONV32 FIN32 GN_STATS32 GN_APPLY32 ATTN32 GEMV32 TAP BUCKET BUCKET_JOIN UPS_SPLIT32 CONV_THIN FIN_GN GEMM_LIGHT32 CONV_BLOCK TEMB_ROW CONV_OUT").split()
 
 
 def summarize(path: str) -> Dict[str, List[float]]:
diff --git a/include/ldm3d.h b/include/ldm3d.h
--- a/include/ldm3d.h
+++ b/include/ldm3d.h
@@ -369,6 +369,10 @@
 size_t ldm_op_conv3d_thin_f32_ws_bytes(int cin, int N, int D, int H, int W, int cout_pad);
 int ldm_op_conv3d_thin_f32(const float* x_f32_ndhwc, int cin, const float* w_packed, const float* bias, float* out_f32_ncdhw, int N, int D, int H,
                            int W, int cout_real, int cout_pad, void* ws, size_t ws_bytes, void* stream);
+int ldm_op_conv3d_out(const void* x_bf16_ndhwc, int cin, const void* w_packed, const float* bias, float* out_f32_ncdhw, int N, int D, int H, int W,
+                      int cout_real, int cout_pad, void* stream);
+int ldm_op_conv3d_out_step(const void* x_bf16_ndhwc, int cin, const void* w_packed, const float* bias, float* out_f32_ncdhw, int N, int D, int H,
+                           int W, int cout_real, int cout_pad, ldm_sampler* sampler, float* x_latent, float* tbuf, int B, void* stream);
 int ldm_op_timestep_embedding(const float* t, float* out, int B, int dim, void* stream);
 int ldm_op_gemv(const void* w, int fp32_weights, const float* bias, const float* x, float* y, int B, int I, int O, int x_stride, int y_stride,
                 int silu_in, void* stream);
```

Result: no change. 529.3, median of 6 (+0.6%).
